# utiasASRL/mm_masking

Hardware: AMD Instinct MI355X
Metric: scan-pairs/s (mask-CNN + 10-iter dICP fwd+bwd) (higher is better)
Workload: dtype bf16; 1 GPU; BASELINE configs[2]: train_icp_weights step fwd+bwd, batch=32 per GPU, 10 dICP iters, point-to-plane Huber, dim=2; 400x3360 polar radar -> GO-CFAR + peaks + polar->Cartesian 640x640 -> U-Net (hand-written NHWC bf16 MFMA kernels, fp32 masters) -> dICP (fp32 points, fp64 normal equations) -> rot+trans+mask_pts loss -> Adam; batch_per_gpu=32, global_batch=32, scan_pts_pad=5120, map_pts=20000, map_pts_pad=20480, icp_iters=10, parallelism=dp1, scene_density=survey (SURVEY.md 8d: 3 500-5 000 valid scan points of 5 120)

## Files before the change

### include/mmk.h

```cpp
#ifndef MMK_H_
#define MMK_H_

#include <stddef.h>
#include <stdint.h>

#ifdef __cplusplus
extern "C" {
#endif

#define MMK_VERSION 502

#define MMK_OK 0
#define MMK_ERR_ARG (-1)
#define MMK_ERR_HIP (-2)
#define MMK_ERR_WORKSPACE (-3)

#define MMK_ICP_PT2PT 0
#define MMK_ICP_PT2PL 1

#define MMK_NN_BRUTE 0
#define MMK_NN_GRID 1

#define MMK_LOSS_NONE 0
#define MMK_LOSS_CAUCHY 1
// ... 175 lines not shown
int mmk_cfar_mask_p(const float *raw, int32_t B, int32_t A, int32_t R, int32_t w2, int32_t guard, int32_t mincol,
                    int32_t maxcol, const float *a_thresh, const float *b_thresh, int32_t per_scan, int32_t diff,
                    float steep_fact, float *mask, void *stream);

size_t mmk_cfar_mask_bwd_p_ws_bytes(int32_t B, int32_t A);
int mmk_cfar_mask_bwd_p(const float *raw, const float *grad_mask , int32_t B, int32_t A, int32_t R, int32_t w2,
                        int32_t guard, int32_t mincol, int32_t maxcol, const float *a_thresh, const float *b_thresh,
                        int32_t per_scan, float steep_fact, float *grad_raw , float *grad_a,
                        float *grad_b , void *workspace, size_t workspace_bytes, void *stream);

size_t mmk_extract_peaks_workspace_bytes(int32_t B, int32_t A, int32_t R, int32_t max_pts);
int mmk_extract_peaks(const float *mask, int32_t B, int32_t A, int32_t R, float res,
                      const float *azimuths , const float *times ,
                      const float *T_ab, int32_t diff, float steep_fact, int32_t max_pts,
                      float *out_pc, int32_t *out_count, void *workspace,
                      size_t workspace_bytes, void *stream);
size_t mmk_extract_peaks_bwd_workspace_bytes(int32_t B, int32_t A, int32_t R, int32_t max_pts);
int mmk_extract_peaks_bwd(const float *mask, int32_t B, int32_t A, int32_t R, float res, const float *azimuths ,
                          const float *T_ab, int32_t diff, float steep_fact, int32_t max_pts,
                          const float *grad_pc , float *grad_mask , void *workspace,
                          size_t workspace_bytes, void *stream);

int mmk_polar_to_cart(const float *polar, const float *azimuths ,
                      const float *range_grid, const float *angle_grid, int32_t B,
                      int32_t A, int32_t R, int32_t W, float radar_resolution,
                      int32_t interpolate_crossover, int32_t fix_wobble, float *cart,
                      void *stream);
int mmk_polar_to_cart_pair(const float *polar, const float *polar2, const float *azimuths,
                           const float *range_grid, const float *angle_grid, int32_t B, int32_t A,
                           int32_t R, int32_t W, float radar_resolution, int32_t interpolate_crossover,
                           int32_t fix_wobble, float *cart, float *cart2, void *stream);

int mmk_cart_to_polar(const double *cart, const double *sin_az, const double *cos_az, const double *range_coords,
                      int32_t B, int32_t A, int32_t R, int32_t H, int32_t W, double cart_resolution, double *polar,
                      void *stream);

size_t mmk_polar_to_cart_bwd_ws_bytes(int32_t B, int32_t A, int32_t R, int32_t W);
int mmk_polar_to_cart_bwd(const float *grad_cart , const float *azimuths , const float *range_grid,
                          const float *angle_grid, int32_t B, int32_t A, int32_t R, int32_t W, float radar_resolution,
                          int32_t interpolate_crossover, int32_t fix_wobble, float *grad_polar , void *ws,
                          size_t ws_bytes, void *stream);

size_t mmk_cart_to_polar_bwd_ws_bytes(int32_t B, int32_t A, int32_t R, int32_t H, int32_t W);
int mmk_cart_to_polar_bwd(const double *grad_polar , const double *sin_az, const double *cos_az,
                          const double *range_coords, int32_t B, int32_t A, int32_t R, int32_t H, int32_t W,
                          double radar_resolution, double cart_resolution, double *grad_cart , void *ws,
                          size_t ws_bytes, void *stream);

int mmk_mask_polar_scan(const float *scan , const float *mask_cart , const double *sin_az,
                        const double *cos_az, const double *range_coords, int32_t B, int32_t A, int32_t R, int32_t H,
                        int32_t W, double cart_resolution, float *out , void *stream);

size_t mmk_mask_polar_scan_bwd_ws_bytes(int32_t B, int32_t A, int32_t R, int32_t H, int32_t W);
int mmk_mask_polar_scan_bwd(const float *grad_out , const float *scan , const float *mask_cart ,
                            const double *sin_az, const double *cos_az, const double *range_coords, int32_t B, int32_t A,
                            int32_t R, int32_t H, int32_t W, double radar_resolution, double cart_resolution,
                            float *grad_scan , float *grad_mask , void *ws, size_t ws_bytes,
                            void *stream);

int mmk_sample_weights_fwd(const float *mask , const float *pc ,
                           int32_t B, int32_t N, int32_t pc_cols, int32_t H, int32_t W,
                           int32_t cart_pixel_width, float cart_resolution,
                           float *weights , void *stream);
size_t mmk_sample_weights_bwd_ws_bytes(int32_t B, int32_t N);
int mmk_sample_weights_bwd(const float *grad_weights , const float *pc, int32_t B,
                           int32_t N, int32_t pc_cols, int32_t H, int32_t W,
                           int32_t cart_pixel_width, float cart_resolution, float *grad_mask,
                           void *ws, size_t ws_bytes, void *stream);
int mmk_sample_weights_bwd_pc(const float *grad_weights , const float *mask , const float *pc,
                              int32_t B, int32_t N, int32_t pc_cols, int32_t H, int32_t W,
                              int32_t cart_pixel_width, float cart_resolution, float *grad_pc, void *stream);

int mmk_sample_weights_polar_fwd(const float *mask , const float *pc , const float *azimuths ,
                                 int32_t B, int32_t N, int32_t pc_cols, int32_t A, int32_t R, float radar_resolution,
                                 int32_t interpolate_crossover, int32_t fix_wobble, float *weights , void *stream);
size_t mmk_sample_weights_polar_bwd_ws_bytes(int32_t B, int32_t N);
int mmk_sample_weights_polar_bwd(const float *grad_weights , const float *pc, const float *azimuths, int32_t B, int32_t N,
                                 int32_t pc_cols, int32_t A, int32_t R, float radar_resolution, int32_t interpolate_crossover,
                                 int32_t fix_wobble, float *grad_mask , void *ws, size_t ws_bytes, void *stream);
int mmk_sample_weights_polar_bwd_pc(const float *grad_weights , const float *mask , const float *pc,
                                    const float *azimuths, int32_t B, int32_t N, int32_t pc_cols, int32_t A, int32_t R,
                                    float radar_resolution, int32_t interpolate_crossover, int32_t fix_wobble,
                                    float *grad_pc , void *stream);

int mmk_host_read_rows(const char *path, int64_t header_bytes, int32_t rows, int32_t row_bytes, int32_t col0,
                       int32_t ncols, int32_t roll, void *dst);
typedef struct mmk_read_job {
    const char *path;
    int64_t header_bytes;
    int32_t rows, row_bytes, col0, ncols, roll, reserved;
    void *dst;
} mmk_read_job;
int mmk_host_read_rows_batch(const mmk_read_job *jobs, int32_t n_jobs, int32_t threads);
int mmk_u8_to_float(const void *in , const float *lut256, int64_t n, float *out, void *stream);

int mmk_weight_stats(const float *weights , const float *pc , int32_t B, int32_t N,
                     int32_t pc_cols, float *partial, float *out, void *stream);

int mmk_bev_raster(const float *pc , int32_t B, int32_t M, int32_t pc_cols,
                   int32_t W, float cart_resolution, float *bev , void *stream);

typedef struct {
    const void *x1;
    const void *x2;
    int32_t C1, C2;
    const void *wpack;
    const float *bias;
    void *y1;
    const void *relu_src1;
    int32_t O1, accumulate1;
    float scale1;
    void *y2;
    const void *relu_src2;
    int32_t O2, accumulate2;
    float scale2;
    int32_t B, H, W;
    int32_t relu;
    float leaky_slope;
    float drop_p;
    uint32_t seed;
    void *pool_y;
    void *pool_arg;
    const void *x1_pool_arg;
    float x1_pool_scale;
} mmk_conv_desc;

size_t mmk_conv_desc_bytes(void);
int32_t mmk_conv3x3_pool_fusable(int32_t cin, int32_t cout, int32_t B, int32_t H, int32_t W);

size_t mmk_conv3x3_packed_elems(int32_t cout, int32_t cin, int32_t transposed);
int mmk_conv3x3_pack_weights(const float *W, int32_t cout, int32_t cin, int32_t transposed,
                             void *packed, void *stream);
int mmk_conv3x3_pack_weights_batch(int32_t n, const float *const *W, const int32_t *cout, const int32_t *cin,
                                   int32_t transposed, void *const *packed, void *stream);
int mmk_conv3x3(const mmk_conv_desc *d, void *stream);
int32_t mmk_conv3x3_wgrad_slices(int32_t cout, int32_t cin, int32_t c1, int32_t B, int32_t H, int32_t W);
int mmk_conv3x3_wgrad_partial(const void *x1, const void *x2, int32_t C1, int32_t C2, const void *g, int32_t cout,
                              int32_t B, int32_t H, int32_t W, float *partials, int32_t accumulate, void *stream);

int mmk_conv_bwd_fused(const void *x, const void *g, const void *wpack_t, float scale, int32_t B, int32_t H, int32_t W,
                       int32_t C, void *dx, float *partials, int32_t accumulate, void *stream);
int mmk_conv_bwd_fused_pooled(const void *x, const void *gy, const void *arg, float pool_scale, const void *wpack_t, float scale,
                              int32_t B, int32_t H, int32_t W, int32_t C, void *dx, float *partials, int32_t accumulate,
                              void *stream);
int mmk_conv3x3_wgrad_partial_pooled(const void *x1, const void *x2, int32_t C1, int32_t C2, const void *gy, const void *arg,
                                     float pool_scale, int32_t cout, int32_t B, int32_t H, int32_t W, float *partials,
                                     int32_t accumulate, void *stream);

int mmk_conv8x16_bwd_fused(const void *x, const void *g, const void *wpack_t, float scale, int32_t B, int32_t H, int32_t W,
                           void *dx, float *partials, int32_t accumulate, void *stream);

int mmk_conv16x8_bwd_fused(const void *x1, const void *x2, const void *g, const void *wpack_t, float scale, int32_t B, int32_t H,
                           int32_t W, void *dx1, void *dx2, float *partials, int32_t accumulate, void *stream);
int mmk_conv3x3_wgrad_unpack_batch(int32_t n, const float *const *src, const int32_t *slices, const int32_t *cout,
                                   const int32_t *cin, float *const *dW, float *const *db, void *stream);

int mmk_channel_minmax(const float *x , int32_t B, int32_t C, int64_t hw, float *part,
                       float *pre , float *minmax , void *stream);
int mmk_channel_meanstd(const float *x , int32_t B, int32_t C, int64_t hw, double *part,
                        float *pre , void *stream);
int mmk_conv_first(const float *x, int32_t cin, const float *W, const float *bias, const float *pre,
                   int32_t B, int32_t H, int32_t Wd, float leaky_slope, void *y, void *stream);
size_t mmk_conv_first_wgrad_ws_bytes(int32_t cin);
int mmk_conv_first_wgrad(const float *x, int32_t cin, const void *g, const float *pre, int32_t B,
                         int32_t H, int32_t Wd, float *dW, float *db, float *ws, size_t ws_bytes, void *stream);
#define MMK_NORM_NONE 0
#define MMK_NORM_MINMAX 1
#define MMK_NORM_STANDARDIZE 2
size_t mmk_conv_first_dgrad_ws_bytes(int32_t cin);
int mmk_conv_first_dgrad(const void *g, int32_t cin, const float *W, const float *x , const float *pre ,
                         const float *minmax , int32_t B, int32_t H, int32_t Wd, float *grad_x, void *ws ,
                         size_t ws_bytes, void *stream);
int mmk_input_norm_bwd(float *grad_x, const float *x, int32_t cin, const float *pre, const float *minmax ,
                       int32_t mode, int32_t B, int32_t H, int32_t Wd, const void *ws, size_t ws_bytes, void *stream);

int mmk_maxpool2_fwd(const void *x, int32_t B, int32_t H, int32_t W, int32_t C, void *y, void *stream);
int mmk_maxpool2_bwd(const void *d, const void *gy, int32_t B, int32_t H, int32_t W, int32_t C, float scale,
                     float leaky_slope, void *gz, void *stream);
int mmk_maxpool2_fwd_arg(const void *x, int32_t B, int32_t H, int32_t W, int32_t C, void *y, void *arg, void *stream);
int mmk_maxpool2_bwd_arg(const void *arg, const void *gy, int32_t B, int32_t H, int32_t W, int32_t C, float scale,
                         void *gz, void *stream);

int mmk_upsample_fwd(const void *x, int32_t B, int32_t Hs, int32_t Ws, int32_t C, int32_t Ho, int32_t Wo, void *y,
                     void *stream);
int mmk_upsample_bwd(const void *gy, int32_t B, int32_t Hs, int32_t Ws, int32_t C, int32_t Ho, int32_t Wo,
                     const void *relu_src, float scale, float leaky_slope, void *gx, void *stream);

#define MMK_FINAL_BWD_WS_FLOATS 16384
int mmk_final_fwd(const void *x, const float *w, const float *bias, int64_t npix, float *mask, void *stream);
int mmk_final_bwd(const void *x, const float *w, const float *mask, const float *gmask, int64_t npix, float scale,
                  float leaky_slope, void *gx, float *dW, float *db, float *ws, void *stream);
int mmk_mask_normalize(const float *mask , int32_t B, int64_t npix_per, float *part,
                       float *mask_n, float *amax, void *stream);
int mmk_final_bwd_normalized(const void *x, const float *w, const float *mask, const float *mask_n,
                             const float *amax, const float *gmask_n, int32_t B, int64_t npix_per,
                             float scale, float leaky_slope, float *part, float *coef, void *gx, float *dW,
                             float *db, float *ws, void *stream);

int mmk_bn_forward_stats(const void *a, int64_t npix, int32_t C, const float *gamma, const float *beta, float eps,
                         float momentum, float *running_mean, float *running_var, float *part, float *stat,
                         float *affine, void *stream);
int mmk_bn_apply(const void *a, int64_t npix, int32_t C, const float *affine, float drop_p, uint32_t seed, void *y,
                 void *stream);
int mmk_bn_backward(const void *gd, const void *d, float drop_scale, const void *a, int64_t npix, int32_t C,
                    const float *stat, const float *affine, const float *gamma, float leaky_slope, int32_t accumulate,
                    float *part, float *coef, float *dgamma, float *dbeta, void *gz, void *stream);

typedef struct {
    int32_t B, H, W, cin;
    const float *x;
    const float *pre;
    const float *const *params;
    float drop_p;
    uint32_t seed;
    float leaky_slope;
    int32_t norm;
    void *workspace;
    size_t workspace_bytes;
    float *mask;
    int32_t keep_full_res;
} mmk_unet_desc;

size_t mmk_unet_workspace_bytes(int32_t B, int32_t H, int32_t W, int32_t cin);
size_t mmk_unet_scratch_bytes(int32_t B, int32_t H, int32_t W, int32_t cin);
int mmk_unet_forward(const mmk_unet_desc *d, void *stream);
int mmk_unet_backward(const mmk_unet_desc *d, const float *gmask, float *const *grads, void *scratch,
                      size_t scratch_bytes, void *stream);
#define MMK_UNET_GRAD_BUCKETS 3
int32_t mmk_unet_grad_bucket(int32_t bucket, int32_t *first_param, int32_t *n_params);
int mmk_unet_backward_buckets(const mmk_unet_desc *d, const float *gmask, float *const *grads, void *scratch,
                              size_t scratch_bytes, void *const *bucket_events, void *stream);
int mmk_unet_backward_input(const mmk_unet_desc *d, const float *gmask, float *const *grads, float *grad_x, int32_t norm_mode,
                            const float *minmax, void *scratch, size_t scratch_bytes, void *const *bucket_events, void *stream);
int mmk_unet_tensor(int32_t B, int32_t H, int32_t W, int32_t cin, int32_t id, size_t *offset, int32_t *h,
                    int32_t *w, int32_t *c);

#ifdef __cplusplus
}
#endif
#endif
```

### mm_masking_amd/_lib.py

```python
import ctypes
import os
import sys
import subprocess

import torch

_HERE = os.path.dirname(os.path.abspath(__file__))
_ROOT = os.path.dirname(_HERE)
SO_PATH = os.environ.get("MMK_LIB", os.path.join(_HERE, "libmmk_hip.so"))
SOURCES = ["mmk_api.hip", "mmk_icp.hip", "mmk_radar.hip", "mmk_unet.hip", "mmk_unet_driver.hip", "mmk_loader.hip", "mmk_loss.hip"]

_lib = None

c_f32p = ctypes.c_void_p
c_vp = ctypes.c_void_p


class MmkError(RuntimeError):
    pass


class ReadJob(ctypes.Structure):
    _fields_ = [("path", ctypes.c_char_p), ("header_bytes", ctypes.c_int64), ("rows", ctypes.c_int32),
                ("row_bytes", ctypes.c_int32), ("col0", ctypes.c_int32), ("ncols", ctypes.c_int32), ("roll", ctypes.c_int32),
                ("reserved", ctypes.c_int32), ("dst", ctypes.c_void_p)]


class IcpParams(ctypes.Structure):
    _fields_ = [("B", ctypes.c_int32), ("N", ctypes.c_int32), ("M", ctypes.c_int32),
                ("tgt_cols", ctypes.c_int32), ("dim", ctypes.c_int32), ("icp_type", ctypes.c_int32),
                ("loss", ctypes.c_int32), ("loss_k", ctypes.c_float), ("trim_dist", ctypes.c_float),
                ("tolerance", ctypes.c_float), ("max_iter", ctypes.c_int32), ("save_state", ctypes.c_int32),
                ("check_every", ctypes.c_int32), ("nn_method", ctypes.c_int32),
                ("trim_steep", ctypes.c_float)]


class IcpSoft(ctypes.Structure):
    _fields_ = [("k", ctypes.c_int32), ("temp", ctypes.c_float)]


class ConvDesc(ctypes.Structure):
    _fields_ = [("x1", ctypes.c_void_p), ("x2", ctypes.c_void_p), ("C1", ctypes.c_int32), ("C2", ctypes.c_int32),
                ("wpack", ctypes.c_void_p), ("bias", ctypes.c_void_p),
                ("y1", ctypes.c_void_p), ("relu_src1", ctypes.c_void_p), ("O1", ctypes.c_int32),
                ("accumulate1", ctypes.c_int32), ("scale1", ctypes.c_float),
                ("y2", ctypes.c_void_p), ("relu_src2", ctypes.c_void_p), ("O2", ctypes.c_int32),
                ("accumulate2", ctypes.c_int32), ("scale2", ctypes.c_float),
                ("B", ctypes.c_int32), ("H", ctypes.c_int32), ("W", ctypes.c_int32), ("relu", ctypes.c_int32),
                ("leaky_slope", ctypes.c_float), ("drop_p", ctypes.c_float), ("seed", ctypes.c_uint32), ("pool_y", ctypes.c_void_p),
                ("pool_arg", ctypes.c_void_p), ("x1_pool_arg", ctypes.c_void_p), ("x1_pool_scale", ctypes.c_float)]


class UNetDesc(ctypes.Structure):
    _fields_ = [("B", ctypes.c_int32), ("H", ctypes.c_int32), ("W", ctypes.c_int32), ("cin", ctypes.c_int32),
                ("x", ctypes.c_void_p), ("pre", ctypes.c_void_p), ("params", ctypes.POINTER(ctypes.c_void_p)),
                ("drop_p", ctypes.c_float), ("seed", ctypes.c_uint32), ("leaky_slope", ctypes.c_float), ("norm", ctypes.c_int32),
                ("workspace", ctypes.c_void_p), ("workspace_bytes", ctypes.c_size_t), ("mask", ctypes.c_void_p),
                ("keep_full_res", ctypes.c_int32)]


FINAL_BWD_WS_FLOATS = 16384
NORM_MODES = {None: 0, "none": 0, "minmax": 1, "standardize": 2}
ICP_TYPES = {"pt2pt": 0, "pt2pl": 1}
LOSSES = {None: 0, "none": 0, "l2": 0, "cauchy": 1, "huber": 2, "geman_mcclure": 3, "welsch": 4}
NN_METHODS = {"brute": 0, "grid": 1}


def build(verbose=False):
    from concurrent.futures import ThreadPoolExecutor
    csrc = os.path.join(_HERE, "csrc")
    srcs = [os.path.join(csrc, s) for s in SOURCES]
    common = [os.path.join(csrc, "mmk_common.h"), os.path.join(csrc, "mmk_unet_shared.h"), os.path.join(_ROOT, "include", "mmk.h")]
    incs = [os.path.join(csrc, f) for f in sorted(os.listdir(csrc)) if f.endswith(".inc")]
    extra = {"mmk_unet.hip": incs, "mmk_loader.hip": incs}
    objdir = os.path.join(csrc, "_obj")
    os.makedirs(objdir, exist_ok=True)
    hipcc = os.environ.get("HIPCC", "/opt/rocm/bin/hipcc")
    flags = ["--offload-arch=gfx950", "-O3", "-std=c++17", "-fPIC", "-ffp-contract=off", "-I", os.path.join(_ROOT, "include")]
    per_file = {"mmk_unet.hip": ["-mllvm", "-amdgpu-mfma-vgpr-form"]}
    jobs, objs = [], []
    for src in srcs:
        obj = os.path.join(objdir, os.path.basename(src)[:-4] + ".o")
        objs.append(obj)
        deps = [src] + common + extra.get(os.path.basename(src), []) + [os.path.abspath(__file__)]
        if not (os.path.exists(obj) and all(os.path.getmtime(obj) >= os.path.getmtime(d) for d in deps)):
            jobs.append([hipcc] + flags + per_file.get(os.path.basename(src), []) + ["-c", src, "-o", obj])
    if not jobs and os.path.exists(SO_PATH) and all(os.path.getmtime(SO_PATH) >= os.path.getmtime(o) for o in objs):
        return SO_PATH

    def run(cmd):
        if verbose:
            print(" ".join(cmd), flush=True)
        try:
            subprocess.check_call(cmd)
        except subprocess.CalledProcessError:
            plain = [c for c in cmd if c not in sum(per_file.values(), [])]
            if len(plain) == len(cmd):
                raise
            print("libmmk_hip: retrying without %s" % " ".join(sorted(set(cmd) - set(plain))), file=sys.stderr, flush=True)
            subprocess.check_call(plain)
    with ThreadPoolExecutor(max_workers=max(1, min(len(jobs), os.cpu_count() or 1))) as ex:
        list(ex.map(run, jobs))
    run([hipcc, "--offload-arch=gfx950", "-shared", "-fPIC", "-o", SO_PATH] + objs)
    return SO_PATH


def _declare(lib):
    i32, f32, sz = ctypes.c_int32, ctypes.c_float, ctypes.c_size_t
    P = ctypes.POINTER(IcpParams)
    S = ctypes.POINTER(IcpSoft)
    sig = {
        "mmk_version": (ctypes.c_int, []),
        "mmk_last_error": (ctypes.c_char_p, []),
        "mmk_icp_params_bytes": (sz, []),
        "mmk_icp_workspace_bytes": (sz, [P]),
        "mmk_icp_forward": (ctypes.c_int, [P] + [c_vp] * 10 + [c_vp, sz, ctypes.POINTER(ctypes.c_int), c_vp]),
        "mmk_icp_backward": (ctypes.c_int, [P] + [c_vp] * 11 + [c_vp, sz, c_vp]),
        "mmk_icp_backward_points_workspace_bytes": (sz, [P, i32]),
        "mmk_icp_backward_points": (ctypes.c_int, [P] + [c_vp] * 13 + [c_vp, sz, c_vp]),
        "mmk_icp_status": (ctypes.c_int, [P, c_vp, sz, c_vp, c_vp]),
        "mmk_icp_forward_hp": (ctypes.c_int, [P] + [c_vp] * 10 + [c_vp, i32, c_vp, sz, ctypes.POINTER(ctypes.c_int), c_vp]),
        "mmk_icp_backward_hp_workspace_bytes": (sz, [P, i32, i32]),
        "mmk_icp_backward_hp": (ctypes.c_int, [P] + [c_vp] * 13 + [c_vp, i32, c_vp, c_vp, sz, c_vp]),
        "mmk_icp_soft_workspace_bytes": (sz, [P, S]),
        "mmk_icp_forward_soft": (ctypes.c_int, [P] + [c_vp] * 10 + [S, c_vp, sz, ctypes.POINTER(ctypes.c_int), c_vp]),
        "mmk_icp_backward_soft_workspace_bytes": (sz, [P, S, i32]),
        "mmk_icp_backward_soft": (ctypes.c_int, [P] + [c_vp] * 13 + [S, c_vp, sz, c_vp]),
        "mmk_icp_forward_soft_t": (ctypes.c_int, [P] + [c_vp] * 10 + [S, c_vp, i32, c_vp, sz, ctypes.POINTER(ctypes.c_int), c_vp]),
        "mmk_icp_backward_soft_t_workspace_bytes": (sz, [P, S, i32, i32]),
        "mmk_icp_backward_soft_t": (ctypes.c_int, [P] + [c_vp] * 13 + [S, c_vp, i32, c_vp, c_vp, sz, c_vp]),
        "mmk_knn_search_workspace_bytes": (sz, [i32, i32, i32, i32]),
        "mmk_knn_search": (ctypes.c_int, [c_vp, c_vp, c_vp, i32, i32, i32, i32, i32, i32, c_vp, c_vp, c_vp, sz, c_vp]),
        "mmk_pose_loss_fwd": (ctypes.c_int, [c_vp, i32, c_vp, c_vp]),
        "mmk_pose_loss_bwd": (ctypes.c_int, [c_vp, i32, c_vp, c_vp, c_vp, c_vp]),
        "mmk_bce_ws_bytes": (sz, []),
        "mmk_bce_mean_fwd": (ctypes.c_int, [c_vp, c_vp, ctypes.c_int64, c_vp, sz, c_vp, c_vp]),
        "mmk_bce_mean_bwd": (ctypes.c_int, [c_vp, c_vp, ctypes.c_int64, c_vp, c_vp, c_vp]),
        "mmk_pose_loss_gt_fwd": (ctypes.c_int, [c_vp, c_vp, i32, c_vp, c_vp]),
        "mmk_pose_loss_gt_bwd": (ctypes.c_int, [c_vp, c_vp, i32, c_vp, c_vp, c_vp, c_vp]),
        "mmk_val_metric": (ctypes.c_int, [c_vp, c_vp, i32, c_vp, c_vp]),
        "mmk_fft_threshold_ws_bytes": (sz, [i32]),
        "mmk_fft_threshold_mask": (ctypes.c_int, [c_vp, i32, ctypes.c_int64, c_vp, sz, c_vp, c_vp]),
        "mmk_bce_fft_threshold_fwd": (ctypes.c_int, [c_vp, c_vp, i32, ctypes.c_int64, c_vp, sz, c_vp, c_vp, c_vp]),
        "mmk_bce_fft_threshold_bwd": (ctypes.c_int, [c_vp, c_vp, i32, ctypes.c_int64, c_vp, c_vp, c_vp, c_vp]),
        "mmk_icp_partials_count": (sz, [P]),
        "mmk_icp_accumulate": (ctypes.c_int, [P] + [c_vp] * 8 + [c_vp]),
        "mmk_icp_solve_update": (ctypes.c_int, [P] + [c_vp] * 7 + [c_vp]),
        "mmk_nn_padded_m": (i32, [i32]),
        "mmk_pack_target": (ctypes.c_int, [c_vp, i32, i32, i32, i32, c_vp, c_vp]),
        "mmk_nn_workspace_bytes": (sz, [i32, i32, i32, i32]),
        "mmk_nn_search": (ctypes.c_int, [c_vp, c_vp, c_vp, i32, i32, i32, i32, c_vp, c_vp, c_vp, sz, c_vp]),
        "mmk_knn_normals_workspace_bytes": (sz, [i32, i32]),
        "mmk_knn_normals": (ctypes.c_int, [c_vp, i32, i32, i32, i32, i32, f32, f32, c_vp, c_vp, c_vp, c_vp, c_vp, c_vp, sz, c_vp]),
        "mmk_nn_profile_begin": (ctypes.c_int, [i32]),
        "mmk_nn_profile_end": (ctypes.c_int, [ctypes.POINTER(ctypes.c_float), i32, ctypes.POINTER(ctypes.c_int32)]),
        "mmk_conv3x3_packed_elems": (sz, [i32, i32, i32]),
        "mmk_conv3x3_pack_weights": (ctypes.c_int, [c_vp, i32, i32, i32, c_vp, c_vp]),
        "mmk_conv3x3_pack_weights_batch": (ctypes.c_int, [i32, c_vp, c_vp, c_vp, i32, c_vp, c_vp]),
        "mmk_conv3x3": (ctypes.c_int, [ctypes.POINTER(ConvDesc), c_vp]),
        "mmk_conv3x3_wgrad_unpack_batch": (ctypes.c_int, [i32, c_vp, c_vp, c_vp, c_vp, c_vp, c_vp, c_vp]),
        "mmk_conv3x3_wgrad_slices": (i32, [i32, i32, i32, i32, i32, i32]),
        "mmk_conv3x3_wgrad_partial": (ctypes.c_int, [c_vp, c_vp, i32, i32, c_vp, i32, i32, i32, i32, c_vp, i32, c_vp]),
        "mmk_conv_bwd_fused": (ctypes.c_int, [c_vp, c_vp, c_vp, ctypes.c_float, i32, i32, i32, i32, c_vp, c_vp, i32, c_vp]),
        "mmk_conv_bwd_fused_pooled": (ctypes.c_int, [c_vp, c_vp, c_vp, f32, c_vp, f32, i32, i32, i32, i32, c_vp, c_vp, i32, c_vp]),
        "mmk_conv3x3_wgrad_partial_pooled": (ctypes.c_int, [c_vp, c_vp, i32, i32, c_vp, c_vp, f32, i32, i32, i32, i32, c_vp, i32, c_vp]),
        "mmk_conv8x16_bwd_fused": (ctypes.c_int, [c_vp, c_vp, c_vp, ctypes.c_float, i32, i32, i32, c_vp, c_vp, i32, c_vp]),
        "mmk_conv16x8_bwd_fused": (ctypes.c_int, [c_vp, c_vp, c_vp, c_vp, ctypes.c_float, i32, i32, i32, c_vp, c_vp, c_vp, i32, c_vp]),
        "mmk_conv_desc_bytes": (sz, []),
        "mmk_conv3x3_pool_fusable": (ctypes.c_int32, [i32, i32, i32, i32, i32]),
        "mmk_channel_minmax": (ctypes.c_int, [c_vp, i32, i32, ctypes.c_int64, c_vp, c_vp, c_vp, c_vp]),
        "mmk_channel_meanstd": (ctypes.c_int, [c_vp, i32, i32, ctypes.c_int64, c_vp, c_vp, c_vp]),
        "mmk_conv_first": (ctypes.c_int, [c_vp, i32, c_vp, c_vp, c_vp, i32, i32, i32, f32, c_vp, c_vp]),
        "mmk_conv_first_wgrad_ws_bytes": (sz, [i32]),
        "mmk_conv_first_wgrad": (ctypes.c_int, [c_vp, i32, c_vp, c_vp, i32, i32, i32, c_vp, c_vp, c_vp, sz, c_vp]),
        "mmk_conv_first_dgrad_ws_bytes": (sz, [i32]),
        "mmk_conv_first_dgrad": (ctypes.c_int, [c_vp, i32, c_vp, c_vp, c_vp, c_vp, i32, i32, i32, c_vp, c_vp, sz, c_vp]),
        "mmk_input_norm_bwd": (ctypes.c_int, [c_vp, c_vp, i32, c_vp, c_vp, i32, i32, i32, i32, c_vp, sz, c_vp]),
        "mmk_maxpool2_fwd": (ctypes.c_int, [c_vp, i32, i32, i32, i32, c_vp, c_vp]),
        "mmk_maxpool2_bwd": (ctypes.c_int, [c_vp, c_vp, i32, i32, i32, i32, f32, f32, c_vp, c_vp]),
        "mmk_maxpool2_fwd_arg": (ctypes.c_int, [c_vp, i32, i32, i32, i32, c_vp, c_vp, c_vp]),
        "mmk_maxpool2_bwd_arg": (ctypes.c_int, [c_vp, c_vp, i32, i32, i32, i32, f32, c_vp, c_vp]),
        "mmk_upsample_fwd": (ctypes.c_int, [c_vp, i32, i32, i32, i32, i32, i32, c_vp, c_vp]),
        "mmk_upsample_bwd": (ctypes.c_int, [c_vp, i32, i32, i32, i32, i32, i32, c_vp, f32, f32, c_vp, c_vp]),
        "mmk_final_fwd": (ctypes.c_int, [c_vp, c_vp, c_vp, ctypes.c_int64, c_vp, c_vp]),
        "mmk_final_bwd": (ctypes.c_int, [c_vp, c_vp, c_vp, c_vp, ctypes.c_int64, f32, f32, c_vp, c_vp, c_vp, c_vp, c_vp]),
        "mmk_mask_normalize": (ctypes.c_int, [c_vp, i32, ctypes.c_int64, c_vp, c_vp, c_vp, c_vp]),
        "mmk_final_bwd_normalized": (ctypes.c_int, [c_vp, c_vp, c_vp, c_vp, c_vp, c_vp, i32, ctypes.c_int64, f32, f32, c_vp, c_vp,
                                                    c_vp, c_vp, c_vp, c_vp, c_vp]),
        "mmk_bn_forward_stats": (ctypes.c_int, [c_vp, ctypes.c_int64, i32, c_vp, c_vp, f32, f32, c_vp, c_vp, c_vp, c_vp, c_vp, c_vp]),
        "mmk_bn_apply": (ctypes.c_int, [c_vp, ctypes.c_int64, i32, c_vp, f32, ctypes.c_uint32, c_vp, c_vp]),
        "mmk_bn_backward": (ctypes.c_int, [c_vp, c_vp, f32, c_vp, ctypes.c_int64, i32, c_vp, c_vp, c_vp, f32, i32, c_vp, c_vp, c_vp,
                                           c_vp, c_vp, c_vp]),
        "mmk_unet_workspace_bytes": (sz, [i32, i32, i32, i32]),
        "mmk_unet_scratch_bytes": (sz, [i32, i32, i32, i32]),
        "mmk_unet_forward": (ctypes.c_int, [ctypes.POINTER(UNetDesc), c_vp]),
        "mmk_unet_backward": (ctypes.c_int, [ctypes.POINTER(UNetDesc), c_vp, ctypes.POINTER(ctypes.c_void_p), c_vp, sz, c_vp]),
        "mmk_unet_backward_buckets": (ctypes.c_int, [ctypes.POINTER(UNetDesc), c_vp, ctypes.POINTER(ctypes.c_void_p), c_vp, sz,
                                                     ctypes.POINTER(ctypes.c_void_p), c_vp]),
        "mmk_unet_backward_input": (ctypes.c_int, [ctypes.POINTER(UNetDesc), c_vp, ctypes.POINTER(ctypes.c_void_p), c_vp, i32, c_vp,
                                                   c_vp, sz, ctypes.POINTER(ctypes.c_void_p), c_vp]),
        "mmk_unet_grad_bucket": (i32, [i32, ctypes.POINTER(i32), ctypes.POINTER(i32)]),
        "mmk_unet_tensor": (ctypes.c_int, [i32, i32, i32, i32, i32, ctypes.POINTER(sz), ctypes.POINTER(i32), ctypes.POINTER(i32),
                                           ctypes.POINTER(i32)]),
        "mmk_cfar_mask": (ctypes.c_int, [c_vp, i32, i32, i32, i32, i32, i32, i32, f32, f32, i32, f32, c_vp, c_vp]),
        "mmk_cfar_mask_bwd": (ctypes.c_int, [c_vp, c_vp, i32, i32, i32, i32, i32, i32, i32, f32, f32, f32, c_vp, c_vp]),
        "mmk_cfar_mask_p": (ctypes.c_int, [c_vp, i32, i32, i32, i32, i32, i32, i32, c_vp, c_vp, i32, i32, f32, c_vp, c_vp]),
        "mmk_cfar_mask_bwd_p_ws_bytes": (sz, [i32, i32]),
        "mmk_cfar_mask_bwd_p": (ctypes.c_int, [c_vp, c_vp, i32, i32, i32, i32, i32, i32, i32, c_vp, c_vp, i32, f32, c_vp, c_vp, c_vp,
                                               c_vp, sz, c_vp]),
        "mmk_extract_peaks_workspace_bytes": (sz, [i32, i32, i32, i32]),
        "mmk_extract_peaks_bwd_workspace_bytes": (sz, [i32, i32, i32, i32]),
        "mmk_extract_peaks_bwd": (ctypes.c_int, [c_vp, i32, i32, i32, f32, c_vp, c_vp, i32, f32, i32, c_vp, c_vp, c_vp, sz, c_vp]),
        "mmk_extract_peaks": (ctypes.c_int, [c_vp, i32, i32, i32, f32, c_vp, c_vp, c_vp, i32, f32, i32, c_vp, c_vp,
                                             c_vp, sz, c_vp]),
        "mmk_polar_to_cart": (ctypes.c_int, [c_vp, c_vp, c_vp, c_vp, i32, i32, i32, i32, f32, i32, i32, c_vp, c_vp]),
        "mmk_polar_to_cart_pair": (ctypes.c_int, [c_vp, c_vp, c_vp, c_vp, c_vp, i32, i32, i32, i32, f32, i32, i32, c_vp, c_vp,
                                                  c_vp]),
        "mmk_cart_to_polar": (ctypes.c_int, [c_vp, c_vp, c_vp, c_vp, i32, i32, i32, i32, i32, ctypes.c_double, c_vp, c_vp]),
        "mmk_polar_to_cart_bwd_ws_bytes": (sz, [i32, i32, i32, i32]),
        "mmk_polar_to_cart_bwd": (ctypes.c_int, [c_vp, c_vp, c_vp, c_vp, i32, i32, i32, i32, f32, i32, i32, c_vp, c_vp, sz, c_vp]),
        "mmk_cart_to_polar_bwd_ws_bytes": (sz, [i32, i32, i32, i32, i32]),
        "mmk_cart_to_polar_bwd": (ctypes.c_int, [c_vp, c_vp, c_vp, c_vp, i32, i32, i32, i32, i32, ctypes.c_double, ctypes.c_double,
                                                 c_vp, c_vp, sz, c_vp]),
        "mmk_mask_polar_scan": (ctypes.c_int, [c_vp, c_vp, c_vp, c_vp, c_vp, i32, i32, i32, i32, i32, ctypes.c_double, c_vp, c_vp]),
        "mmk_mask_polar_scan_bwd_ws_bytes": (sz, [i32, i32, i32, i32, i32]),
        "mmk_mask_polar_scan_bwd": (ctypes.c_int, [c_vp, c_vp, c_vp, c_vp, c_vp, c_vp, i32, i32, i32, i32, i32, ctypes.c_double,
                                                   ctypes.c_double, c_vp, c_vp, c_vp, sz, c_vp]),
        "mmk_sample_weights_fwd": (ctypes.c_int, [c_vp, c_vp, i32, i32, i32, i32, i32, i32, f32, c_vp, c_vp]),
        "mmk_host_read_rows": (ctypes.c_int, [ctypes.c_char_p, ctypes.c_int64, i32, i32, i32, i32, i32, c_vp]),
        "mmk_host_read_rows_batch": (ctypes.c_int, [ctypes.POINTER(ReadJob), i32, i32]),
        "mmk_u8_to_float": (ctypes.c_int, [c_vp, c_vp, ctypes.c_int64, c_vp, c_vp]),
        "mmk_sample_weights_bwd_ws_bytes": (sz, [i32, i32]),
        "mmk_sample_weights_bwd": (ctypes.c_int, [c_vp, c_vp, i32, i32, i32, i32, i32, i32, f32, c_vp, c_vp, sz, c_vp]),
        "mmk_sample_weights_bwd_pc": (ctypes.c_int, [c_vp, c_vp, c_vp, i32, i32, i32, i32, i32, i32, f32, c_vp, c_vp]),
        "mmk_sample_weights_polar_fwd": (ctypes.c_int, [c_vp, c_vp, c_vp, i32, i32, i32, i32, i32, f32, i32, i32, c_vp, c_vp]),
        "mmk_sample_weights_polar_bwd_ws_bytes": (sz, [i32, i32]),
        "mmk_sample_weights_polar_bwd": (ctypes.c_int, [c_vp, c_vp, c_vp, i32, i32, i32, i32, i32, f32, i32, i32, c_vp, c_vp, sz,
                                                        c_vp]),
        "mmk_sample_weights_polar_bwd_pc": (ctypes.c_int, [c_vp, c_vp, c_vp, c_vp, i32, i32, i32, i32, i32, f32, i32, i32, c_vp,
                                                           c_vp]),
        "mmk_weight_stats": (ctypes.c_int, [c_vp, c_vp, i32, i32, i32, c_vp, c_vp, c_vp]),
        "mmk_bev_raster": (ctypes.c_int, [c_vp, i32, i32, i32, i32, f32, c_vp, c_vp]),
    }
    for name, (res, args) in sig.items():
        fn = getattr(lib, name)
        fn.restype = res
        fn.argtypes = args
    return sig


EXPORTED = None


def lib():
    global _lib, EXPORTED
    if _lib is None:
        if not os.path.exists(SO_PATH):
            raise MmkError("libmmk_hip.so is not built: run `python -c 'import __graft_entry__ as g; g.build()'` "
                           "(hipcc --offload-arch=gfx950).  The HIP path has no CPU fallback.")
        try:
            loaded = ctypes.CDLL(SO_PATH)
        except OSError as e:
            raise MmkError("cannot load %s: %s" % (SO_PATH, e)) from e
        EXPORTED = _declare(loaded)
        if loaded.mmk_conv_desc_bytes() != ctypes.sizeof(ConvDesc):
            raise MmkError("%s: mmk_conv_desc is %d bytes, the ctypes mirror %d" % (SO_PATH, loaded.mmk_conv_desc_bytes(), ctypes.sizeof(ConvDesc)))
        if loaded.mmk_icp_params_bytes() != ctypes.sizeof(IcpParams):
            raise MmkError("%s: mmk_icp_params is %d bytes, the ctypes mirror %d" % (SO_PATH, loaded.mmk_icp_params_bytes(), ctypes.sizeof(IcpParams)))
        _lib = loaded
    return _lib


def check(rc):
    if rc != 0:
        raise MmkError("libmmk_hip: %s (code %d)" % (lib().mmk_last_error().decode(errors="replace"), rc))


def stream_ptr(device=None):
    if device is not None:
        idx = device.index if isinstance(device, torch.device) else int(device)
        if idx is not None and idx != torch.cuda.current_device():
            raise MmkError("tensors live on cuda:%d but the current HIP device is cuda:%d: call torch.cuda.set_device() "
                           "(one process per GPU) or wrap the call in `with torch.cuda.device(...)`"
                           % (idx, torch.cuda.current_device()))
    return ctypes.c_void_p(torch.cuda.current_stream(device).cuda_stream)


def ptr(t, dtype=None, name="tensor"):
    if t is None:
        return ctypes.c_void_p(0)
    if not t.is_cuda:
        raise MmkError("%s must live on a HIP device (got %s); the kernels have no CPU path" % (name, t.device))
    if dtype is not None and t.dtype != dtype:
        raise MmkError("%s must be %s (got %s)" % (name, dtype, t.dtype))
    if not t.is_contiguous():
        raise MmkError("%s must be contiguous" % name)
    return ctypes.c_void_p(t.data_ptr())


_ws_cache = {}


def workspace(nbytes, device, tag):
    key = (device.index, torch.cuda.current_stream(device).cuda_stream, tag)
    buf = _ws_cache.get(key)
    if buf is None or buf.numel() < nbytes:
        buf = torch.empty(max(int(nbytes), 1), dtype=torch.uint8, device=device)
        _ws_cache[key] = buf
    return buf


def dev_f32(t, device):
    return t.detach().to(device=device, dtype=torch.float32).contiguous()
```

### mm_masking_amd/csrc/mmk_unet.hip

```cpp
#include <math.h>
#include <stdlib.h>

#include <algorithm>
#include <type_traits>

#include "mmk_common.h"
#include "mmk_unet_shared.h"

namespace {

using namespace mmku;

__device__ __forceinline__ unsigned cvt_pk_bf16(float lo, float hi)
{
    unsigned r;
    asm("v_cvt_pk_bf16_f32 %0, %1, %2" : "=v"(r) : "v"(lo), "v"(hi));
    return r;
}
__device__ __forceinline__ unsigned pk_relu_bf16(unsigned x)
{
    unsigned r;
    asm("v_pk_max_i16 %0, %1, 0" : "=v"(r) : "v"(x));
    return r;
}
// ... 1634 lines not shown
        {
            if (t + t_step < t_end) {
                ld_tx += adv_tx;
                const int cx = ld_tx >= tiles_x ? 1 : 0;
                ld_tx -= cx ? tiles_x : 0;
                ld_ty += adv_ty + cx;
                const int cy = ld_ty >= tiles_y ? 1 : 0;
                ld_ty -= cy ? tiles_y : 0;
                ld_b += adv_b + cy;
            }
            load_tile(ld_b, ld_ty, ld_tx);
        }
        i32x2 fa[2][2 * MT], fb[2][2 * NTW];
#define WG_ISSUE(R, BUF)                                                                                 \
    {                                                                                                    \
        _Pragma("unroll") for (int m = 0; m < MT; ++m) {                                                 \
            fa[BUF][2 * m] = (m == 0) ? tr_read_o<((R) * TW * PG) * 2>(g_ad)                             \
                           : (m == 1) ? tr_read_o<((R) * TW * PG + 16) * 2>(g_ad)                        \
                           : (m == 2) ? tr_read_o<((R) * TW * PG + 32) * 2>(g_ad)                        \
                                      : tr_read_o<((R) * TW * PG + 48) * 2>(g_ad);                       \
            fa[BUF][2 * m + 1] = (m == 0) ? tr_read_o<((R) * TW * PG + 16 * PG) * 2>(g_ad)                \
                               : (m == 1) ? tr_read_o<((R) * TW * PG + 16 + 16 * PG) * 2>(g_ad)           \
                               : (m == 2) ? tr_read_o<((R) * TW * PG + 32 + 16 * PG) * 2>(g_ad)           \
                                          : tr_read_o<((R) * TW * PG + 48 + 16 * PG) * 2>(g_ad);          \
        }                                                                                                \
        _Pragma("unroll") for (int n = 0; n < NTW; ++n) {                                                \
            fb[BUF][2 * n] = tr_read_o<((R) * WT * PK) * 2>(b_ad[n]);                                    \
            fb[BUF][2 * n + 1] = tr_read_o<((R) * WT * PK + 16 * PK) * 2>(b_ad[n]);                       \
        }                                                                                                \
    }
#define WG_CONSUME(BUF)                                                                                  \
    {                                                                                                    \
        _Pragma("unroll") for (int m = 0; m < MT; ++m) {                                                 \
            const bf16x8 af = frag_from(fa[BUF][2 * m], fa[BUF][2 * m + 1]);                             \
             \
             \
            _Pragma("unroll") for (int n = 0; n < NTW; ++n)                                              \
                acc[m][n] = __builtin_amdgcn_mfma_f32_16x16x32_bf16(af, frag_from(fb[BUF][2 * n], fb[BUF][2 * n + 1]), acc[m][n], 0, 0, 0); \
            accb[m] = __builtin_amdgcn_mfma_f32_16x16x32_bf16(af, ones, accb[m], 0, 0, 0);               \
        }                                                                                                \
    }
#define WG_STEP(R)                                                                                       \
    {                                                                                                    \
        asm volatile("s_waitcnt lgkmcnt(0)" ::: "memory");                                               \
        __builtin_amdgcn_sched_barrier(0);                                                               \
        if ((R) + 1 < TH) WG_ISSUE(((R) + 1 < TH ? (R) + 1 : 0), ((R) + 1) & 1);                         \
        __builtin_amdgcn_sched_barrier(0);                                                               \
        WG_CONSUME((R) & 1);                                                                             \
    }
        WG_ISSUE(0, 0);
        WG_STEP(0) WG_STEP(1) WG_STEP(2) WG_STEP(3) WG_STEP(4) WG_STEP(5) WG_STEP(6) WG_STEP(7)
        static_assert(TH == 8, "WG_STEP expansion above covers 8 tile rows");
#undef WG_STEP
#undef WG_CONSUME
#undef WG_ISSUE
    }

    const size_t pstride = (size_t)9 * a.COUT * a.CIN + a.COUT;
#pragma unroll
    for (int m = 0; m < MT; ++m) {
#pragma unroll
        for (int rr = 0; rr < 4; ++rr) {
            const int co = group * CM + m * 16 + g4 * 4 + rr;
            if (co >= a.COUT) continue;
#pragma unroll
            for (int n = 0; n < NTW; ++n) {
                const int nt = wv + 4 * n;
                if (nt >= NTT) continue;
                int tap, ci;
                if (CK >= 16) {
                    tap = nt / (CK / 16);
                    ci = chunk * CK + (nt % (CK / 16)) * 16 + i16;
                } else {
                    tap = 2 * nt + (i16 >> 3);
                    ci = i16 & 7;
                }
                if (tap < 9) {
                    float *d = a.partials + (size_t)blockIdx.x * pstride + ((size_t)tap * a.COUT + co) * a.CIN + ci;
                    *d = a.acc_partials ? *d + acc[m][n][rr] : acc[m][n][rr];
                }
            }
            if (wv == 0 && chunk == 0 && i16 == 0) {
                float *d = a.partials + (size_t)blockIdx.x * pstride + (size_t)9 * a.COUT * a.CIN + co;
                *d = a.acc_partials ? *d + accb[m][rr] : accb[m][rr];
            }
        }
    }
}

constexpr size_t wgrad_smem(int CX, int CG)
{
    return ((size_t)(HT * WT + 8) * wg_pitch(CX) + (size_t)(TH * TW + 8) * wg_pitch(CG)) * sizeof(bf16);
}

template <int CK, int CM, bool G8>
int wgrad_spatial(int cout, int cin, int B, int H, int W)
{
    constexpr int cap = (CK <= 16 && CM == 16) ? 4 : 8;
    int per_cu = 0;
    if (blocks_per_cu<conv3x3_wgrad_kernel<CK, CM, G8>>(CONV_THREADS, wgrad_smem(CK, G8 ? 8 : CM), cap, &per_cu) != hipSuccess) return -1;
    const int tiles = ((W + TW - 1) / TW) * ((H + TH - 1) / TH) * B;
    const int chunks = cin / CK, groups = (cout + CM - 1) / CM;
    int spatial = (256 * per_cu) / (chunks * groups);
    spatial = spatial < 1 ? 1 : (spatial > tiles ? tiles : spatial);
    return spatial >= 8 ? (spatial & ~7) : spatial;
}

template <int CK, int CM, bool G8, bool POOLG = false>
int launch_wgrad(const WgradArgs &a, hipStream_t st)
{
    constexpr size_t smem = wgrad_smem(CK, G8 ? 8 : CM);
    const int spatial = wgrad_spatial<CK, CM, G8>(a.COUT, a.CIN, a.B, a.H, a.W);
    if (spatial < 1) {
        mmk::set_error("mmk_conv3x3_wgrad: occupancy query failed");
        return MMK_ERR_HIP;
    }
    const int chunks = a.CIN / CK, groups = (a.COUT + CM - 1) / CM;
    if constexpr (POOLG)
        MMK_CHECK_HIP((raise_lds_limit<conv3x3_wgrad_kernel<CK, CM, G8, true>>(smem > 64 * 1024, smem)));
    hipLaunchKernelGGL((conv3x3_wgrad_kernel<CK, CM, G8, POOLG>), dim3(spatial, chunks, groups), dim3(CONV_THREADS), smem, st, a);
    MMK_LAUNCH_CHECK();
    return MMK_OK;
}


struct BwdFusedArgs {
    const bf16 *x, *x2;
    const bf16 *g;
    const bf16 *wpack_t;
    bf16 *dx, *dx2;
    float scale;
    int masked;
    int accumulate_dx;
    int B, H, W;
    float *partials;
    int acc_partials;
    const unsigned *g_arg = nullptr;
    float g_scale = 1.f;
};

BwdFusedArgs bwd_fused_args(const void *x, const void *x2, const void *g, const void *wpack_t, void *dx, void *dx2, float scale,
                            int masked, int B, int H, int W, float *partials, int accumulate)
{
    BwdFusedArgs a = {};
    a.x = (const bf16 *)x; a.x2 = (const bf16 *)x2; a.g = (const bf16 *)g; a.wpack_t = (const bf16 *)wpack_t;
    a.dx = (bf16 *)dx; a.dx2 = (bf16 *)dx2; a.scale = scale; a.masked = masked;
    a.B = B; a.H = H; a.W = W; a.partials = partials; a.acc_partials = accumulate;
    return a;
}

template <int CX, int CG, bool POOLG = false>
__global__ __launch_bounds__(CONV_THREADS) void conv_bwd_fused_kernel(const BwdFusedArgs a)
{
    static_assert((CX == 8 || CX == 16) && (CG == 8 || CG == 16), "thin layers");
    constexpr int NTT = CX == 8 ? 5 : 9;
    constexpr int NTW = (NTT + 3) / 4;
    constexpr int NS = CG == 8 ? 3 : 5;
    constexpr int NT = 4;
    constexpr int GX = CX / 8, GG = CG / 8;
    __shared__ __attribute__((aligned(16))) bf16 x_tile[(HT * WT + 8) * CX];
    __shared__ __attribute__((aligned(16))) bf16 g_tile[(HT * WT + 8) * CG];
    __shared__ __attribute__((aligned(16))) bf16 w_lds[NS * 64 * 8];

    const int tid = threadIdx.x, lane = tid & 63;
    const int wv = __builtin_amdgcn_readfirstlane(tid >> 6);
    const int tiles_x = (a.W + TW - 1) / TW, tiles_y = (a.H + TH - 1) / TH;
    const int tpi = tiles_x * tiles_y;
    const int total_tiles = tpi * a.B;
    const int i16 = lane & 15, g4 = lane >> 4, q = i16 >> 2, pp = i16 & 3;
    const bool split = a.x2 != nullptr;

    f32x4 acc[NTW], accb = {0.f, 0.f, 0.f, 0.f};
#pragma unroll
    for (int n = 0; n < NTW; ++n) acc[n] = (f32x4){0.f, 0.f, 0.f, 0.f};
    bf16x8 ones;
#pragma unroll
    for (int j = 0; j < 8; ++j) ones[j] = (bf16)1.0f;
    unsigned b_ad[NTW];
#pragma unroll
    for (int n = 0; n < NTW; ++n) {
        const int nt = wv + 4 * n;
        int tap = CX == 8 ? 2 * nt + (pp >> 1) : nt;
        const int col = CX == 8 ? 4 * (pp & 1) : 4 * pp;
        tap = tap > 8 ? 8 : tap;
        const int ty = tap / 3, tx = tap % 3;
        b_ad[n] = lds_addr(x_tile) + (unsigned)((((ty * WT) + 4 * g4 + q + tx) * CX + col) * 2);
    }
    const unsigned g_ad = lds_addr(g_tile) + (unsigned)(((WT + 1 + 4 * g4 + q) * CG + 4 * pp) * 2);

    int d_lane[NS];
#pragma unroll
    for (int ks = 0; ks < NS; ++ks) {
        int tap = CG == 8 ? 4 * ks + (lane >> 4) : 2 * ks + (lane >> 5);
        const int ch = CG == 8 ? 0 : 8 * ((lane >> 4) & 1);
        tap = tap > 8 ? 8 : tap;
        d_lane[ks] = ((2 * wv + tap / 3) * WT + (lane & 15) + tap % 3) * CG + ch;
    }
    const int n8 = lane >> 4;
    const int lrow8 = 2 * wv + (n8 >> 1), lcol8 = (n8 & 1) * 16 + (lane & 15);
    const int lpix8 = lrow8 * a.W + lcol8;
    const int s_off8 = ((lrow8 + 1) * WT + lcol8 + 1) * CX;
    int o_pix[NT], s_off[NT];
#pragma unroll
    for (int n = 0; n < NT; ++n) {
        const int r = 2 * wv + (n >> 1), c = (n & 1) * 16 + (lane & 15);
        o_pix[n] = r * a.W + c;
        s_off[n] = ((r + 1) * WT + c + 1) * CX + (lane >> 4) * 4;
    }
    bf16 *const o_base = (a.dx2 != nullptr) ? ((lane >> 5) ? a.dx2 : a.dx) + ((lane >> 4) & 1) * 4 : a.dx + (lane >> 4) * 4;
    const int o_stride = (a.dx2 != nullptr) ? 8 : 16;
    for (int i = tid; i < NS * 64; i += CONV_THREADS) reinterpret_cast<u32x4 *>(w_lds)[i] = reinterpret_cast<const u32x4 *>(a.wpack_t)[i];

    constexpr int NX = HT * WT * GX, NG = HT * WT * GG;
    constexpr int RX = (NX + CONV_THREADS - 1) / CONV_THREADS, RG = (NG + CONV_THREADS - 1) / CONV_THREADS;
    constexpr int PH = TH / 2 + 2, PW = TW / 2 + 2, NPG = PH * PW * GG;
    constexpr int NRG = POOLG ? (NPG + CONV_THREADS - 1) / CONV_THREADS : RG;
    u32x4 rx[RX], rg[NRG];
    unsigned rc[POOLG ? NRG : 1];
    const int Hp = a.H >> 1, Wp = a.W >> 1;
    auto load_tile = [&](int b, int tyi, int txi) {
        int tv = tid;
        asm volatile("" : "+v"(tv));
        const int tx0 = txi * TW, ty0 = tyi * TH;
        const int pix0 = (b * a.H + ty0) * a.W + tx0;
#pragma unroll
        for (int i = 0; i < RX; ++i) {
            int gi = tv + i * CONV_THREADS;
            gi = gi < NX ? gi : NX - 1;
            const int pix = gi / GX, half = gi % GX;
            const int dy = pix / WT - 1, dx = pix % WT - 1;
            const bool ok = (unsigned)(ty0 + dy) < (unsigned)a.H && (unsigned)(tx0 + dx) < (unsigned)a.W;
            const long po = pix0 + dy * a.W + dx;
            const bf16 *src = split ? (half ? a.x2 : a.x) + po * 8 : a.x + po * CX + half * 8;
            rx[i] = *(ok ? reinterpret_cast<const u32x4 *>(src) : &g_zero16);
        }
        if constexpr (POOLG) {
#pragma unroll
            for (int i = 0; i < NRG; ++i) {
                int gi = tv + i * CONV_THREADS;
                gi = gi < NPG ? gi : NPG - 1;
                const int pp = gi / GG, gc = gi % GG;
                const int py = (ty0 >> 1) + pp / PW - 1, px = (tx0 >> 1) + pp % PW - 1;
                const bool ok = (unsigned)py < (unsigned)Hp && (unsigned)px < (unsigned)Wp;
                const long e = (long)((b * Hp + py) * Wp + px) * GG + gc;
                rg[i] = *(ok ? reinterpret_cast<const u32x4 *>(a.g + e * 8) : &g_zero16);
                rc[i] = *(ok ? a.g_arg + e : reinterpret_cast<const unsigned *>(&g_zero16));
            }
        } else {
#pragma unroll
            for (int i = 0; i < RG; ++i) {
                int gi = tv + i * CONV_THREADS;
                gi = gi < NG ? gi : NG - 1;
                const int pix = gi / GG, gc = gi % GG;
                const int dy = pix / WT - 1, dx = pix % WT - 1;
                const bool ok = (unsigned)(ty0 + dy) < (unsigned)a.H && (unsigned)(tx0 + dx) < (unsigned)a.W;
                rg[i] = *(ok ? reinterpret_cast<const u32x4 *>(a.g + (long)(pix0 + dy * a.W + dx) * CG + gc * 8) : &g_zero16);
            }
        }
    };
    auto store_tile = [&]() {
        int tv = tid;
        asm volatile("" : "+v"(tv));
#pragma unroll
        for (int i = 0; i < RX; ++i) {
            const int gi = tv + i * CONV_THREADS;
            if (gi < NX) *reinterpret_cast<u32x4 *>(x_tile + (size_t)gi * 8) = rx[i];
        }
        if constexpr (POOLG) {
#pragma unroll
            for (int i = 0; i < NRG; ++i) {
                const int gi = tv + i * CONV_THREADS;
                const int pp = gi / GG, gc = gi % GG;
                const int r0 = 2 * (pp / PW) - 1, c0 = 2 * (pp % PW) - 1;
                poolg_write(g_tile + (r0 * WT + c0) * CG + gc * 8, CG, WT * CG, r0, c0, HT, WT, gi < NPG, rg[i], rc[i], a.g_scale);
            }
        } else {
#pragma unroll
            for (int i = 0; i < RG; ++i) {
                const int gi = tv + i * CONV_THREADS;
                if (gi < NG) *reinterpret_cast<u32x4 *>(g_tile + (size_t)gi * 8) = rg[i];
            }
        }
    };

    int t_first, t_step, t_end;
    if ((gridDim.x & 7) == 0) {
        const int per_xcd = (total_tiles + 7) / 8;
        const int xcd = blockIdx.x & 7;
        t_first = xcd * per_xcd + ((int)blockIdx.x >> 3);
        t_step = (int)gridDim.x >> 3;
        t_end = min(total_tiles, (xcd + 1) * per_xcd);
    } else {
        t_first = blockIdx.x; t_step = gridDim.x; t_end = total_tiles;
    }
    const int adv_tx = t_step % tiles_x, adv_ty = (t_step / tiles_x) % tiles_y, adv_b = t_step / tpi;
    int ld_b = t_first / tpi, ld_ty = (t_first % tpi) / tiles_x, ld_tx = t_first % tiles_x;
    int cb = ld_b, cty = ld_ty, ctx = ld_tx;
    if (t_first < t_end) {
        load_tile(ld_b, ld_ty, ld_tx);
        store_tile();
    }
    __syncthreads();
    for (int t = t_first; t < t_end; t += t_step) {
        const int b = cb;
        const int tx0 = ctx * TW, ty0 = cty * TH;
        const int pix0 = (b * a.H + ty0) * a.W + tx0;
        const bool ok8 = (ty0 + lrow8) < a.H && (tx0 + lcol8) < a.W;
        u32x4 e8_acc = {0u, 0u, 0u, 0u};
        if constexpr (CX == 8) e8_acc = *((ok8 && a.accumulate_dx) ? reinterpret_cast<const u32x4 *>(a.dx + (long)(pix0 + lpix8) * 8) : &g_zero16);
        {
            if (t + t_step < t_end) {
                ld_tx += adv_tx;
                const int cx = ld_tx >= tiles_x ? 1 : 0;
                ld_tx -= cx ? tiles_x : 0;
                ld_ty += adv_ty + cx;
                const int cy = ld_ty >= tiles_y ? 1 : 0;
                ld_ty -= cy ? tiles_y : 0;
                ld_b += adv_b + cy;
            }
            load_tile(ld_b, ld_ty, ld_tx);
            cb = ld_b; cty = ld_ty; ctx = ld_tx;
        }
        i32x2 fa[2][2], fb[2][2 * NTW];
#define BF_ISSUE(R, BUF)                                                                     \
    {                                                                                        \
        fa[BUF][0] = tr_read_o<((R) * WT * CG) * 2>(g_ad);                                   \
        fa[BUF][1] = tr_read_o<((R) * WT * CG + 16 * CG) * 2>(g_ad);                         \
        _Pragma("unroll") for (int n = 0; n < NTW; ++n) {                                    \
            fb[BUF][2 * n] = tr_read_o<((R) * WT * CX) * 2>(b_ad[n]);                        \
            fb[BUF][2 * n + 1] = tr_read_o<((R) * WT * CX + 16 * CX) * 2>(b_ad[n]);          \
        }                                                                                    \
    }
#define BF_CONSUME(BUF)                                                                      \
    {                                                                                        \
        const bf16x8 af = frag_from(fa[BUF][0], fa[BUF][1]);                                 \
        _Pragma("unroll") for (int n = 0; n < NTW; ++n)                                      \
            acc[n] = __builtin_amdgcn_mfma_f32_16x16x32_bf16(af, frag_from(fb[BUF][2 * n], fb[BUF][2 * n + 1]), acc[n], 0, 0, 0); \
        accb = __builtin_amdgcn_mfma_f32_16x16x32_bf16(af, ones, accb, 0, 0, 0);             \
    }
#define BF_STEP(R)                                                                           \
    {                                                                                        \
        asm volatile("s_waitcnt lgkmcnt(0)" ::: "memory");                                   \
        __builtin_amdgcn_sched_barrier(0);                                                   \
        if ((R) + 1 < TH) BF_ISSUE(((R) + 1 < TH ? (R) + 1 : 0), ((R) + 1) & 1);             \
        __builtin_amdgcn_sched_barrier(0);                                                   \
        BF_CONSUME((R) & 1);                                                                 \
    }
        BF_ISSUE(0, 0);
        BF_STEP(0) BF_STEP(1) BF_STEP(2) BF_STEP(3) BF_STEP(4) BF_STEP(5) BF_STEP(6) BF_STEP(7)
        static_assert(TH == 8, "BF_STEP expansion above covers 8 tile rows");
#undef BF_STEP
#undef BF_CONSUME
#undef BF_ISSUE
        f32x4 dacc[NT];
#pragma unroll
        for (int n = 0; n < NT; ++n) dacc[n] = (f32x4){0.f, 0.f, 0.f, 0.f};
#pragma unroll
        for (int ks = 0; ks < NS; ++ks) {
            const bf16 *bl = g_tile + d_lane[ks];
            bf16x8 bf[NT];
#pragma unroll
            for (int n = 0; n < NT; ++n) bf[n] = *reinterpret_cast<const bf16x8 *>(bl + ((n >> 1) * WT + (n & 1) * 16) * CG);
            const bf16x8 af = *reinterpret_cast<const bf16x8 *>(w_lds + ((size_t)(ks * 64 + lane)) * 8);
#pragma unroll
            for (int n = 0; n < NT; ++n) dacc[n] = __builtin_amdgcn_mfma_f32_16x16x32_bf16(af, bf[n], dacc[n], 0, 0, 0);
        }
        u32x4 e8_src = {0u, 0u, 0u, 0u};
        bf16x4 e_src[NT];
        if constexpr (CX == 8) {
            e8_src = *reinterpret_cast<const u32x4 *>(x_tile + s_off8);
        } else {
#pragma unroll
            for (int n = 0; n < NT; ++n) e_src[n] = *reinterpret_cast<const bf16x4 *>(x_tile + s_off[n]);
        }
#pragma unroll
        for (int i = 0; i < RX; ++i) asm volatile("" : "+v"(rx[i]));
#pragma unroll
        for (int i = 0; i < NRG; ++i) asm volatile("" : "+v"(rg[i]));
        if constexpr (POOLG) {
#pragma unroll
            for (int i = 0; i < NRG; ++i) asm volatile("" : "+v"(rc[i]));
        }
        if constexpr (CX == 8) {
            float v8[8];
#pragma unroll
            for (int r = 0; r < 4; ++r) {
                const auto s01 = __builtin_amdgcn_permlane16_swap(__float_as_uint(dacc[0][r]), __float_as_uint(dacc[1][r]), false, false);
                const auto s23 = __builtin_amdgcn_permlane16_swap(__float_as_uint(dacc[2][r]), __float_as_uint(dacc[3][r]), false, false);
                const auto lo = __builtin_amdgcn_permlane32_swap(s01[0], s23[0], false, false);
                const auto hi = __builtin_amdgcn_permlane32_swap(s01[1], s23[1], false, false);
                v8[r] = __uint_as_float(lo[0]);
                v8[4 + r] = __uint_as_float(hi[0]);
            }
            float sv[8], av[8];
            unpack8(e8_src, sv);
            unpack8(e8_acc, av);
#pragma unroll
            for (int r = 0; r < 8; ++r) {
                const float v = fmaxf(v8[r] + 0.f, -INFINITY);
                const float masked = (sv[r] > 0.f) ? v * a.scale : 0.f;
                v8[r] = masked + av[r];
            }
            u32x4 *dst8 = ok8 ? reinterpret_cast<u32x4 *>(a.dx + (long)(pix0 + lpix8) * 8) : reinterpret_cast<u32x4 *>(g_sink16);
            *dst8 = pack8(v8);
        } else {
#pragma unroll
            for (int n = 0; n < NT; ++n) {
                const bool okp = (ty0 + 2 * wv + (n >> 1)) < a.H && (tx0 + (n & 1) * 16 + (lane & 15)) < a.W;
                bf16x4 outv;
#pragma unroll
                for (int r = 0; r < 4; ++r) {
                    const float v = fmaxf(dacc[n][r] + 0.f, -INFINITY);
                    const float masked = ((float)e_src[n][r] > 0.f) ? v * a.scale : 0.f;
                    outv[r] = (bf16)(a.masked ? masked + 0.f : v);
                }
                bf16x4 *dst = okp ? reinterpret_cast<bf16x4 *>(o_base + (long)(pix0 + o_pix[n]) * o_stride) : reinterpret_cast<bf16x4 *>(g_sink16);
                *dst = outv;
            }
        }
        if (t + t_step >= t_end) break;
        __syncthreads();
        store_tile();
        __syncthreads();
    }

    constexpr size_t pstride = (size_t)9 * CG * CX + CG;
#pragma unroll
    for (int rr = 0; rr < 4; ++rr) {
        const int co = g4 * 4 + rr;
        if (co >= CG) continue;
#pragma unroll
        for (int n = 0; n < NTW; ++n) {
            const int nt = wv + 4 * n;
            if (nt >= NTT) continue;
            const int tap = CX == 8 ? 2 * nt + (i16 >> 3) : nt;
            const int ci = CX == 8 ? (i16 & 7) : i16;
            if (tap < 9) {
                float *d = a.partials + (size_t)blockIdx.x * pstride + ((size_t)tap * CG + co) * CX + ci;
                *d = a.acc_partials ? *d + acc[n][rr] : acc[n][rr];
            }
        }
        if (wv == 0 && i16 == 0) {
            float *d = a.partials + (size_t)blockIdx.x * pstride + (size_t)9 * CG * CX + co;
            *d = a.acc_partials ? *d + accb[rr] : accb[rr];
        }
    }
}

constexpr int WGD_THREADS = 512;

template <bool POOLG = false>
__global__ __launch_bounds__(WGD_THREADS) void conv3x3_wgrad_deep_kernel(const WgradArgs a)
{
    constexpr int CK = 64, CM = 64, PK = wg_pitch(64), PG = wg_pitch(64);
    extern __shared__ __attribute__((aligned(16))) unsigned char smem[];
    bf16 *x_tile = reinterpret_cast<bf16 *>(smem);
    bf16 *g_tile = x_tile + (HT * WT + 8) * PK;

    const int tid = threadIdx.x, lane = tid & 63;
    const int wv = __builtin_amdgcn_readfirstlane(tid >> 6);
    const int wm = wv >> 2, wc = wv & 3;
    const int chunk = blockIdx.y, group = blockIdx.z;
    const int tiles_x = (a.W + TW - 1) / TW, tiles_y = (a.H + TH - 1) / TH;
    const int tpi = tiles_x * tiles_y;
    const int total_tiles = tpi * a.B;
    const int i16 = lane & 15, g4 = lane >> 4, q = i16 >> 2, pp = i16 & 3;

    f32x4 acc[3][3][2];
    f32x4 accb[2];
#pragma unroll
    for (int m = 0; m < 2; ++m) {
        accb[m] = (f32x4){0.f, 0.f, 0.f, 0.f};
#pragma unroll
        for (int ty = 0; ty < 3; ++ty)
#pragma unroll
            for (int tx = 0; tx < 3; ++tx) acc[ty][tx][m] = (f32x4){0.f, 0.f, 0.f, 0.f};
    }
    bf16x8 ones;
#pragma unroll
    for (int j = 0; j < 8; ++j) ones[j] = (bf16)1.0f;

    const unsigned xb0 = lds_addr(x_tile) + (unsigned)(((4 * g4 + q) * PK + wc * 16 + 4 * pp) * 2);
    const unsigned gb0 = lds_addr(g_tile) + (unsigned)(((4 * g4 + q) * PG + wm * 32 + 4 * pp) * 2);

    constexpr int GPP = CK / 8;
    constexpr int NIN = HT * WT * GPP;
    constexpr int RIN = (NIN + WGD_THREADS - 1) / WGD_THREADS;
    constexpr int GPG = CM / 8;
    constexpr int NG = TH * TW * GPG;
    constexpr int RG = (NG + WGD_THREADS - 1) / WGD_THREADS;
    constexpr int PWG = TW / 2, NPG = (TH / 2) * PWG * GPG;
    constexpr int NRG = POOLG ? (NPG + WGD_THREADS - 1) / WGD_THREADS : RG;
    u32x4 rin[RIN], rg[NRG];
    unsigned rc[POOLG ? NRG : 1];
    const int Hp = a.H >> 1, Wp = a.W >> 1;
    auto load_tile = [&](int b, int tyi, int txi) {
        int tv = tid;
        asm volatile("" : "+v"(tv));
        const int tx0 = txi * TW, ty0 = tyi * TH;
        const int c0 = chunk * CK;
        const bool in1 = c0 < a.C1;
        const bf16 *xb = in1 ? a.x1 : a.x2;
        const int xc = in1 ? a.C1 : a.C2, cb = in1 ? c0 : c0 - a.C1;
#pragma unroll
        for (int i = 0; i < RIN; ++i) {
            int gi = tv + i * WGD_THREADS;
            gi = gi < NIN ? gi : NIN - 1;
            const int pix = gi / GPP, gc = gi % GPP;
            const int yy = ty0 + pix / WT - 1, xx = tx0 + pix % WT - 1;
            const bool ok = yy >= 0 && yy < a.H && xx >= 0 && xx < a.W;
            const size_t p = ((size_t)b * a.H + yy) * a.W + xx;
            const u32x4 *sp = ok ? reinterpret_cast<const u32x4 *>(xb + p * xc + cb + gc * 8) : &g_zero16;
            rin[i] = *sp;
        }
        if constexpr (POOLG) {
#pragma unroll
            for (int i = 0; i < NRG; ++i) {
                int gi = tv + i * WGD_THREADS;
                gi = gi < NPG ? gi : NPG - 1;
                const int pp = gi / GPG, gc = gi % GPG;
                const int py = (ty0 >> 1) + pp / PWG, px = (tx0 >> 1) + pp % PWG;
                const bool ok = py < Hp && px < Wp;
                const size_t e = (((size_t)b * Hp + py) * Wp + px) * (a.COUT >> 3) + ((group * CM) >> 3) + gc;
                rg[i] = *(ok ? reinterpret_cast<const u32x4 *>(a.g + e * 8) : &g_zero16);
                rc[i] = *(ok ? a.g_arg + e : reinterpret_cast<const unsigned *>(&g_zero16));
            }
        } else {
#pragma unroll
        for (int i = 0; i < RG; ++i) {
            int gi = tv + i * WGD_THREADS;
            gi = gi < NG ? gi : NG - 1;
            const int pix = gi / GPG, gc = gi % GPG;
            const int yy = ty0 + pix / TW, xx = tx0 + pix % TW;
            const bool ok = yy < a.H && xx < a.W;
            const size_t p = ((size_t)b * a.H + yy) * a.W + xx;
            const u32x4 *sp = ok ? reinterpret_cast<const u32x4 *>(a.g + p * a.COUT + group * CM + gc * 8) : &g_zero16;
            rg[i] = *sp;
        }
        }
    };
    auto store_tile = [&]() {
        int tv = tid;
        asm volatile("" : "+v"(tv));
#pragma unroll
        for (int i = 0; i < RIN; ++i) {
            const int gi = tv + i * WGD_THREADS;
            if (gi < NIN) *reinterpret_cast<u32x4 *>(x_tile + (size_t)(gi / GPP) * PK + (gi % GPP) * 8) = rin[i];
        }
        if constexpr (POOLG) {
#pragma unroll
            for (int i = 0; i < NRG; ++i) {
                const int gi = tv + i * WGD_THREADS;
                const int pp = gi / GPG, gc = gi % GPG;
                const int r0 = 2 * (pp / PWG), c0 = 2 * (pp % PWG);
                poolg_write(g_tile + (r0 * TW + c0) * PG + gc * 8, PG, TW * PG, r0, c0, TH, TW, gi < NPG, rg[i], rc[i], a.g_scale);
            }
        } else {
#pragma unroll
        for (int i = 0; i < RG; ++i) {
            const int gi = tv + i * WGD_THREADS;
            if (gi < NG) *reinterpret_cast<u32x4 *>(g_tile + (size_t)(gi / GPG) * PG + (gi % GPG) * 8) = rg[i];
        }
        }
    };

    int t_first, t_step, t_end;
    if ((gridDim.x & 7) == 0) {
        const int per_xcd = (total_tiles + 7) / 8;
        const int xcd = blockIdx.x & 7;
        t_first = xcd * per_xcd + ((int)blockIdx.x >> 3);
        t_step = (int)gridDim.x >> 3;
        t_end = min(total_tiles, (xcd + 1) * per_xcd);
    } else {
        t_first = blockIdx.x; t_step = gridDim.x; t_end = total_tiles;
    }
    const int adv_tx = t_step % tiles_x, adv_ty = (t_step / tiles_x) % tiles_y, adv_b = t_step / tpi;
    int ld_b = t_first / tpi, ld_ty = (t_first % tpi) / tiles_x, ld_tx = t_first % tiles_x;
    if (t_first < t_end) load_tile(ld_b, ld_ty, ld_tx);
    for (int t = t_first; t < t_end; t += t_step) {
        __syncthreads();
        store_tile();
        __syncthreads();
        {
            if (t + t_step < t_end) {
                ld_tx += adv_tx;
                const int cx = ld_tx >= tiles_x ? 1 : 0;
                ld_tx -= cx ? tiles_x : 0;
                ld_ty += adv_ty + cx;
                const int cy = ld_ty >= tiles_y ? 1 : 0;
                ld_ty -= cy ? tiles_y : 0;
                ld_b += adv_b + cy;
            }
            load_tile(ld_b, ld_ty, ld_tx);
        }
        i32x2 fb[2][3][2], fa[4][2][2];
#define WGD_ISSUE(RHO)                                                                                   \
    {                                                                                                    \
// ... 1531 lines not shown

bool chan_ok(int c) { return c == 8 || c == 16 || c == 32 || (c >= 64 && c % 64 == 0); }

}

#ifdef MMK_DEEP_STAMPS
extern "C" int mmk_debug_deep_stamps(unsigned long long *buf)
{
    MMK_CHECK_HIP(hipMemcpyToSymbol(HIP_SYMBOL(g_deep_stamp_buf), &buf, sizeof(buf)));
    return MMK_OK;
}
#endif

extern "C" size_t mmk_conv3x3_packed_elems(int32_t cout, int32_t cin, int32_t transposed)
{
    const int co_n = transposed ? cin : cout, ci_n = transposed ? cout : cin;
    if (!chan_ok(co_n) || !chan_ok(ci_n)) return 0;
    const int CK = conv_ck(ci_n), CM = conv_cm(ci_n, co_n);
    const int groups = (co_n + CM - 1) / CM, chunks = ci_n / CK;
    return (size_t)groups * chunks * ksteps(CK) * (CM / 16) * 512;
}

extern "C" int mmk_conv3x3_pack_weights(const float *W, int32_t cout, int32_t cin, int32_t transposed, void *packed,
                                        void *stream)
{
    MMK_REQUIRE(W && packed, "mmk_conv3x3_pack_weights: NULL pointer");
    const size_t total = mmk_conv3x3_packed_elems(cout, cin, transposed);
    MMK_REQUIRE(total > 0, "mmk_conv3x3_pack_weights: unsupported channel counts %d -> %d", cin, cout);
    hipLaunchKernelGGL(pack_conv_weights_kernel, dim3((unsigned)((total + 255) / 256)), dim3(256), 0, (hipStream_t)stream, W,
                       cout, cin, transposed, (bf16 *)packed, (int)total);
    MMK_LAUNCH_CHECK();
    return MMK_OK;
}

extern "C" int mmk_conv3x3_pack_weights_batch(int32_t n, const float *const *W, const int32_t *cout, const int32_t *cin,
                                              int32_t transposed, void *const *packed, void *stream)
{
    MMK_REQUIRE(n >= 1 && W && cout && cin && packed, "mmk_conv3x3_pack_weights_batch: bad argument");
    for (int base = 0; base < n; base += PACK_BATCH_MAX) {
        PackBatch pb;
        const int m = std::min(PACK_BATCH_MAX, n - base);
        size_t most = 0;
        for (int i = 0; i < PACK_BATCH_MAX; ++i) {
            const int k = base + (i < m ? i : 0);
            MMK_REQUIRE(W[k] && packed[k], "mmk_conv3x3_pack_weights_batch: NULL pointer (layer %d)", k);
            const size_t total = mmk_conv3x3_packed_elems(cout[k], cin[k], transposed);
            MMK_REQUIRE(total > 0 && total < ((size_t)1 << 31), "mmk_conv3x3_pack_weights_batch: unsupported channel counts %d -> %d",
                        cin[k], cout[k]);
            pb.W[i] = W[k]; pb.out[i] = (bf16 *)packed[k]; pb.cout[i] = cout[k]; pb.cin[i] = cin[k];
            pb.total[i] = (int)total;
            most = std::max(most, total);
        }
        pb.transposed = transposed;
        const unsigned bx = (unsigned)std::min<size_t>((most + 255) / 256, 256);
        hipLaunchKernelGGL(pack_conv_weights_batch_kernel, dim3(bx, m), dim3(256), 0, (hipStream_t)stream, pb);
        MMK_LAUNCH_CHECK();
    }
    return MMK_OK;
}

extern "C" int mmk_conv3x3(const mmk_conv_desc *d, void *stream)
{
    MMK_REQUIRE(d != nullptr, "mmk_conv3x3: NULL descriptor");
    MMK_REQUIRE(d->x1 && d->wpack && (d->y1 || (d->pool_y && d->pool_arg)), "mmk_conv3x3: NULL pointer");
    MMK_REQUIRE(d->pool_arg == nullptr || d->pool_y != nullptr, "mmk_conv3x3: pool_arg needs pool_y");
    MMK_REQUIRE(d->B >= 1 && d->H >= 1 && d->W >= 1, "mmk_conv3x3: bad shape");
    const int cin = d->C1 + d->C2, cout = d->O1 + d->O2;
    MMK_REQUIRE(d->C1 % 8 == 0 && d->C2 % 8 == 0 && (d->C2 == 0 || d->x2), "mmk_conv3x3: bad input split %d+%d", d->C1, d->C2);
    MMK_REQUIRE(d->O1 % 8 == 0 && d->O2 % 8 == 0 && (d->O2 == 0 || d->y2), "mmk_conv3x3: bad output split %d+%d", d->O1, d->O2);
    MMK_REQUIRE(chan_ok(cin) && chan_ok(cout), "mmk_conv3x3: unsupported channel counts %d -> %d", cin, cout);
    MMK_REQUIRE(dropout_prob_ok(d->drop_p), "mmk_conv3x3: dropout probability %g out of range (it is quantised to thr / 65536, thr <= 65535)", (double)d->drop_p);
    ConvArgs a;
    a.x1 = (const bf16 *)d->x1; a.x2 = (const bf16 *)d->x2; a.C1 = d->C1; a.C2 = d->C2;
    a.wpack = (const bf16 *)d->wpack; a.bias = d->bias;
    a.o1 = {(bf16 *)d->y1, (const bf16 *)d->relu_src1, d->O1, d->accumulate1, d->scale1};
    a.o2 = {(bf16 *)d->y2, (const bf16 *)d->relu_src2, d->O2, d->accumulate2, d->scale2};
    a.B = d->B; a.H = d->H; a.W = d->W; a.CIN = cin; a.COUT = cout;
    MMK_REQUIRE(d->leaky_slope >= 0.f && d->leaky_slope <= 1.f, "mmk_conv3x3: leaky_slope must be in [0, 1]");
    a.relu = d->relu; a.slope = d->leaky_slope; a.drop_p = d->drop_p; a.seed = d->seed;
    a.pool_y = (bf16 *)d->pool_y;
    a.pool_arg = (unsigned char *)d->pool_arg;
    a.x1_pool_arg = (const unsigned *)d->x1_pool_arg;
    a.x1_pool_scale = d->x1_pool_scale;
    return dispatch_conv(a, (hipStream_t)stream);
}

extern "C" size_t mmk_conv_desc_bytes(void) { return sizeof(mmk_conv_desc); }

extern "C" int32_t mmk_conv3x3_pool_fusable(int32_t cin, int32_t cout, int32_t B, int32_t H, int32_t W)
{
    return pool_fusable(cin, cout, B, H, W) ? 1 : 0;
}

extern "C" int mmk_conv3x3_wgrad_unpack_batch(int32_t n, const float *const *src, const int32_t *slices, const int32_t *cout,
                                              const int32_t *cin, float *const *dW, float *const *db, void *stream)
{
    MMK_REQUIRE(n >= 1 && src && cout && cin && dW, "mmk_conv3x3_wgrad_unpack_batch: bad argument");
    for (int base = 0; base < n; base += PACK_BATCH_MAX) {
        UnpackBatch ub;
        const int m = std::min(PACK_BATCH_MAX, n - base);
        int most = 0;
        for (int i = 0; i < PACK_BATCH_MAX; ++i) {
            const int k = base + (i < m ? i : 0);
            MMK_REQUIRE(src[k] && dW[k] && cout[k] >= 1 && cin[k] >= 1, "mmk_conv3x3_wgrad_unpack_batch: bad layer %d", k);
            ub.src[i] = src[k]; ub.dW[i] = dW[k]; ub.cout[i] = cout[k]; ub.cin[i] = cin[k];
            ub.slices[i] = slices ? slices[k] : 0;
            ub.db[i] = (db && ub.slices[i] > 0) ? db[k] : nullptr;
            const int total = cout[k] * cin[k] * 9 + (ub.slices[i] > 0 ? cout[k] : 0);
            const int epb = 4 * (256 / unpack_groups(total));
            most = std::max(most, (total + epb - 1) / epb);
        }
        const unsigned bx = (unsigned)std::min(most, 2048);
        hipLaunchKernelGGL(unpack_wgrad_batch_kernel, dim3(bx, m), dim3(256), 0, (hipStream_t)stream, ub);
        MMK_LAUNCH_CHECK();
    }
    return MMK_OK;
}

template <int CX, int CG, bool POOLG = false>
int launch_bwd_fused(const BwdFusedArgs &a, int c1, hipStream_t st)
{
    const int spatial = wgrad_slices(CG, CX, c1, a.B, a.H, a.W);
    if (spatial < 1) {
        mmk::set_error("fused backward: occupancy query failed");
        return MMK_ERR_HIP;
    }
    hipLaunchKernelGGL((conv_bwd_fused_kernel<CX, CG, POOLG>), dim3(spatial), dim3(CONV_THREADS), 0, st, a);
    MMK_LAUNCH_CHECK();
    return MMK_OK;
}

extern "C" int mmk_conv_bwd_fused(const void *x, const void *g, const void *wpack_t, float scale, int32_t B, int32_t H, int32_t W,
                                  int32_t C, void *dx, float *partials, int32_t accumulate, void *stream)
{
    MMK_REQUIRE(x && g && wpack_t && dx && partials, "mmk_conv_bwd_fused: NULL pointer");
    MMK_REQUIRE(B >= 1 && H >= 2 && W >= 2 && (C == 8 || C == 16), "mmk_conv_bwd_fused: bad shape (8 or 16 channels)");
    MMK_REQUIRE((size_t)B * H * W * C < ((size_t)1 << 31), "mmk_conv_bwd_fused: tensor too large for 32-bit offsets");
    const BwdFusedArgs a = bwd_fused_args(x, nullptr, g, wpack_t, dx, nullptr, scale, 1, B, H, W, partials, accumulate);
    return C == 8 ? launch_bwd_fused<8, 8>(a, 8, (hipStream_t)stream) : launch_bwd_fused<16, 16>(a, 16, (hipStream_t)stream);
}

extern "C" int mmk_conv_bwd_fused_pooled(const void *x, const void *gy, const void *arg, float pool_scale, const void *wpack_t, float scale,
                                         int32_t B, int32_t H, int32_t W, int32_t C, void *dx, float *partials, int32_t accumulate,
                                         void *stream)
{
    MMK_REQUIRE(x && gy && arg && wpack_t && dx && partials, "mmk_conv_bwd_fused_pooled: NULL pointer");
    MMK_REQUIRE(B >= 1 && H >= 2 && W >= 2 && C == 16, "mmk_conv_bwd_fused_pooled: bad shape (16 channels)");
    MMK_REQUIRE((size_t)B * H * W * C < ((size_t)1 << 31), "mmk_conv_bwd_fused_pooled: tensor too large for 32-bit offsets");
    BwdFusedArgs a = bwd_fused_args(x, nullptr, gy, wpack_t, dx, nullptr, scale, 1, B, H, W, partials, accumulate);
    a.g_arg = (const unsigned *)arg; a.g_scale = pool_scale;
    return launch_bwd_fused<16, 16, true>(a, 16, (hipStream_t)stream);
}

extern "C" int mmk_conv8x16_bwd_fused(const void *x, const void *g, const void *wpack_t, float scale, int32_t B, int32_t H, int32_t W,
                                      void *dx, float *partials, int32_t accumulate, void *stream)
{
    MMK_REQUIRE(x && g && wpack_t && dx && partials, "mmk_conv8x16_bwd_fused: NULL pointer");
    MMK_REQUIRE(B >= 1 && H >= 2 && W >= 2, "mmk_conv8x16_bwd_fused: bad shape");
    MMK_REQUIRE((size_t)B * H * W * 16 < ((size_t)1 << 31), "mmk_conv8x16_bwd_fused: tensor too large for 32-bit offsets");
    BwdFusedArgs a = bwd_fused_args(x, nullptr, g, wpack_t, dx, nullptr, scale, 1, B, H, W, partials, accumulate);
    a.accumulate_dx = 1;
    return launch_bwd_fused<8, 16>(a, 8, (hipStream_t)stream);
}

extern "C" int mmk_conv16x8_bwd_fused(const void *x1, const void *x2, const void *g, const void *wpack_t, float scale, int32_t B,
                                      int32_t H, int32_t W, void *dx1, void *dx2, float *partials, int32_t accumulate, void *stream)
{
    MMK_REQUIRE(x1 && g && wpack_t && dx1 && partials, "mmk_conv16x8_bwd_fused: NULL pointer");
    MMK_REQUIRE((x2 == nullptr) == (dx2 == nullptr), "mmk_conv16x8_bwd_fused: x2 and dx2 go together (both NULL: one 16-channel input / unmasked output)");
    MMK_REQUIRE(B >= 1 && H >= 2 && W >= 2, "mmk_conv16x8_bwd_fused: bad shape");
    MMK_REQUIRE((size_t)B * H * W * 16 < ((size_t)1 << 31), "mmk_conv16x8_bwd_fused: tensor too large for 32-bit offsets");
    const BwdFusedArgs a = bwd_fused_args(x1, x2, g, wpack_t, dx1, dx2, scale, x2 != nullptr, B, H, W, partials, accumulate);
    return launch_bwd_fused<16, 8>(a, x2 ? 8 : 16, (hipStream_t)stream);
}

extern "C" int32_t mmk_conv3x3_wgrad_slices(int32_t cout, int32_t cin, int32_t c1, int32_t B, int32_t H, int32_t W)
{
    if (B < 1 || H < 1 || W < 1 || !chan_ok(cin) || !chan_ok(cout)) return 0;
    const int ns = wgrad_slices(cout, cin, c1, B, H, W);
    return ns < 0 ? 0 : ns;
}

namespace {
int wgrad_partial(const char *who, const void *x1, const void *x2, int C1, int C2, const void *g, const void *arg, float pool_scale,
                  bool pooled, int cout, int B, int H, int W, float *partials, int accumulate, void *stream)
{
    MMK_REQUIRE(x1 && g && partials && (arg || !pooled), "%s: NULL pointer", who);
    MMK_REQUIRE(B >= 1 && H >= (pooled ? 2 : 1) && W >= (pooled ? 2 : 1), "%s: bad shape", who);
    const int cin = C1 + C2;
    MMK_REQUIRE(C1 % 8 == 0 && C2 % 8 == 0 && (C2 == 0 || x2), "%s: bad input split %d+%d", who, C1, C2);
    MMK_REQUIRE(chan_ok(cin) && chan_ok(cout), "%s: unsupported channel counts %d -> %d", who, cin, cout);
    WgradArgs a;
    a.x1 = (const bf16 *)x1; a.x2 = (const bf16 *)x2; a.C1 = C1; a.C2 = C2; a.g = (const bf16 *)g;
    a.B = B; a.H = H; a.W = W; a.CIN = cin; a.COUT = cout;
    a.partials = partials; a.acc_partials = accumulate;
    a.g_arg = (const unsigned *)arg; a.g_scale = pool_scale;
    return dispatch_wgrad(a, (hipStream_t)stream);
}
}

extern "C" int mmk_conv3x3_wgrad_partial(const void *x1, const void *x2, int32_t C1, int32_t C2, const void *g, int32_t cout,
                                         int32_t B, int32_t H, int32_t W, float *partials, int32_t accumulate, void *stream)
{
    return wgrad_partial("mmk_conv3x3_wgrad_partial", x1, x2, C1, C2, g, nullptr, 1.f, false, cout, B, H, W, partials, accumulate, stream);
}

extern "C" int mmk_conv3x3_wgrad_partial_pooled(const void *x1, const void *x2, int32_t C1, int32_t C2, const void *gy, const void *arg,
                                                float pool_scale, int32_t cout, int32_t B, int32_t H, int32_t W, float *partials,
                                                int32_t accumulate, void *stream)
{
    return wgrad_partial("mmk_conv3x3_wgrad_partial_pooled", x1, x2, C1, C2, gy, arg, pool_scale, true, cout, B, H, W, partials, accumulate,
                         stream);
}

extern "C" int mmk_bn_forward_stats(const void *a, int64_t npix, int32_t C, const float *gamma, const float *beta, float eps,
                                    float momentum, float *running_mean, float *running_var, float *part, float *stat, float *affine,
                                    void *stream)
{
    MMK_REQUIRE(a && gamma && beta && part && stat && affine, "mmk_bn_forward_stats: NULL pointer");
    MMK_REQUIRE(npix >= 1 && chan_ok(C) && C <= 2048, "mmk_bn_forward_stats: bad shape (npix %lld, C %d)", (long long)npix, C);
    MMK_REQUIRE((running_mean == nullptr) == (running_var == nullptr), "mmk_bn_forward_stats: running_mean / running_var go together");
    hipStream_t st = (hipStream_t)stream;
    const int per = 256 / (C / 8);
    const int nblk = (int)std::min<int64_t>(BN_BLOCKS, (npix + per - 1) / per);
    hipLaunchKernelGGL(bn_stats_kernel, dim3(nblk), dim3(256), 0, st, (const bf16 *)a, (size_t)npix, C, part);
    MMK_LAUNCH_CHECK();
    hipLaunchKernelGGL(bn_finalize_kernel, dim3((C + 63) / 64), dim3(64), 0, st, part, nblk, C, (double)npix, gamma, beta, eps, momentum,
                       running_mean, running_var, stat, affine);
    MMK_LAUNCH_CHECK();
    return MMK_OK;
}

extern "C" int mmk_bn_apply(const void *a, int64_t npix, int32_t C, const float *affine, float drop_p, uint32_t seed, void *y,
                            void *stream)
{
    MMK_REQUIRE(a && affine && y, "mmk_bn_apply: NULL pointer");
    MMK_REQUIRE(npix >= 1 && chan_ok(C), "mmk_bn_apply: bad shape");
    MMK_REQUIRE(dropout_prob_ok(drop_p), "mmk_bn_apply: dropout probability %g out of range (it is quantised to thr / 65536, thr <= 65535)", (double)drop_p);
    const size_t ngran = (size_t)npix * (C / 8);
    hipLaunchKernelGGL(bn_apply_kernel, dim3((unsigned)std::min<size_t>((ngran + 255) / 256, 8192)), dim3(256), 0, (hipStream_t)stream,
                       (const bf16 *)a, ngran, C, affine, drop_p, seed, (bf16 *)y);
    MMK_LAUNCH_CHECK();
    return MMK_OK;
}

extern "C" int mmk_bn_backward(const void *gd, const void *d, float drop_scale, const void *a, int64_t npix, int32_t C,
                               const float *stat, const float *affine, const float *gamma, float leaky_slope, int32_t accumulate,
                               float *part, float *coef, float *dgamma, float *dbeta, void *gz, void *stream)
{
    MMK_REQUIRE(gd && a && coef && gz, "mmk_bn_backward: NULL pointer");
    MMK_REQUIRE(npix >= 1 && chan_ok(C) && C <= 2048, "mmk_bn_backward: bad shape");
    hipStream_t st = (hipStream_t)stream;
    const size_t ngran = (size_t)npix * (C / 8);
    const unsigned gb = (unsigned)std::min<size_t>((ngran + 255) / 256, 8192);
    if (stat != nullptr) {
        MMK_REQUIRE(gamma && part && dgamma && dbeta, "mmk_bn_backward: NULL pointer (training mode)");
        const int per = 256 / (C / 8);
        const int nblk = (int)std::min<int64_t>(BN_BLOCKS, (npix + per - 1) / per);
        hipLaunchKernelGGL(bn_bwd_reduce_kernel, dim3(nblk), dim3(256), 0, st, (const bf16 *)gd, (const bf16 *)d, drop_scale,
                           (const bf16 *)a, (size_t)npix, C, stat, part);
        MMK_LAUNCH_CHECK();
        hipLaunchKernelGGL(bn_bwd_finalize_kernel, dim3((C + 63) / 64), dim3(64), 0, st, part, nblk, C, (double)npix, gamma, stat,
                           accumulate, coef, dgamma, dbeta);
        MMK_LAUNCH_CHECK();
    } else {
        MMK_REQUIRE(affine != nullptr, "mmk_bn_backward: evaluation mode needs the affine (scale, shift) pairs");
        hipLaunchKernelGGL(bn_eval_coef_kernel, dim3((C + 63) / 64), dim3(64), 0, st, affine, C, coef);
        MMK_LAUNCH_CHECK();
    }
    hipLaunchKernelGGL(bn_bwd_apply_kernel, dim3(gb), dim3(256), 0, st, (const bf16 *)gd, (const bf16 *)d, drop_scale, (const bf16 *)a,
                       ngran, C, stat, coef, leaky_slope, (bf16 *)gz);
    MMK_LAUNCH_CHECK();
    return MMK_OK;
}

static unsigned nblk(size_t n, int t) { return (unsigned)((n + t - 1) / t); }

extern "C" int mmk_channel_minmax(const float *x, int32_t B, int32_t C, int64_t hw, float *part, float *pre, float *minmax,
                                  void *stream)
{
    MMK_REQUIRE(x && part && pre && B >= 1 && C >= 1 && C <= 65535 && hw >= 1, "mmk_channel_minmax: bad argument");
    hipStream_t st = (hipStream_t)stream;
    hipLaunchKernelGGL(channel_minmax_partial_kernel, dim3(MM_BLOCKS, C), dim3(256), 0, st, x, B, C, (size_t)hw, part);
    MMK_LAUNCH_CHECK();
    hipLaunchKernelGGL(channel_minmax_final_kernel, dim3(C), dim3(256), 0, st, part, C, pre, minmax);
    MMK_LAUNCH_CHECK();
    return MMK_OK;
}

extern "C" int mmk_channel_meanstd(const float *x, int32_t B, int32_t C, int64_t hw, double *part, float *pre, void *stream)
{
    MMK_REQUIRE(x && part && pre && B >= 1 && C >= 1 && C <= 65535 && hw >= 1, "mmk_channel_meanstd: bad argument");
    hipStream_t st = (hipStream_t)stream;
    hipLaunchKernelGGL(channel_moment_partial_kernel<false>, dim3(MM_BLOCKS, C), dim3(256), 0, st, x, B, C, (size_t)hw, part);
    MMK_LAUNCH_CHECK();
    hipLaunchKernelGGL(channel_moment_partial_kernel<true>, dim3(MM_BLOCKS, C), dim3(256), 0, st, x, B, C, (size_t)hw, part);
    MMK_LAUNCH_CHECK();
    hipLaunchKernelGGL(channel_meanstd_final_kernel, dim3(C), dim3(256), 0, st, (const double *)part, (size_t)B * (size_t)hw, pre);
    MMK_LAUNCH_CHECK();
    return MMK_OK;
}

extern "C" int mmk_conv_first(const float *x, int32_t cin, const float *W, const float *bias, const float *pre, int32_t B,
                              int32_t H, int32_t Wd, float leaky_slope, void *y, void *stream)
{
    MMK_REQUIRE(x && W && y, "mmk_conv_first: NULL pointer");
    MMK_REQUIRE(leaky_slope >= 0.f && leaky_slope < 1.f, "mmk_conv_first: leaky_slope must be in [0, 1)");
    MMK_REQUIRE(cin >= 1 && cin <= 4 && B >= 1 && H >= 1 && Wd >= 1, "mmk_conv_first: bad shape (cin must be 1..4)");
    const size_t npix = (size_t)B * H * Wd;
    if (Wd % 4 == 0 && npix < (1u << 31)) {
        const unsigned blocks = (unsigned)std::min<size_t>((npix / 4 + 255) / 256, 4096);
        if (leaky_slope > 0.f)
            hipLaunchKernelGGL(conv_first_x4_kernel<true>, dim3(blocks), dim3(256), 0, (hipStream_t)stream, x, cin, W, bias, pre, B, H, Wd,
                               leaky_slope, (bf16 *)y);
        else
            hipLaunchKernelGGL(conv_first_x4_kernel<false>, dim3(blocks), dim3(256), 0, (hipStream_t)stream, x, cin, W, bias, pre, B, H, Wd,
                               leaky_slope, (bf16 *)y);
        MMK_LAUNCH_CHECK();
        return MMK_OK;
    }
    const unsigned blocks = (unsigned)std::min<size_t>((npix + 255) / 256, 8192);
    hipLaunchKernelGGL(conv_first_kernel, dim3(blocks), dim3(256), 0, (hipStream_t)stream, x, cin, W, bias, pre, B, H, Wd, leaky_slope,
                       (bf16 *)y);
    MMK_LAUNCH_CHECK();
    return MMK_OK;
}
// ... 264 lines not shown
```

### mm_masking_amd/csrc/mmk_unet_driver.hip

```cpp
#include <stdlib.h>
#include <string.h>

#include "mmk_common.h"
#include "mmk_unet_shared.h"

namespace {

using mmku::dropout_prob_ok;

constexpr int NCONV = 23;
const int ENC_CH[6] = {8, 16, 32, 64, 128, 256};

struct Tens {
    size_t off = 0;
    int h = 0, w = 0, c = 0;
};

struct Plan {
    int B, H, W, cin;
    int rh[6], rw[6];
    int cout[NCONV], cinn[NCONV];
    Tens a_enc[6], d_enc[6], t[6];
    size_t t_arg[6];
    Tens u[5], a1[5], d1[5], a2[5], d2[5];
// ... 18 lines not shown
        off += bytes;
        return o;
    }
    Tens tens(int B, int h, int w, int c)
    {
        Tens t;
        t.h = h; t.w = w; t.c = c;
        t.off = take((size_t)B * h * w * c * 2);
        return t;
    }
};

bool make_plan(Plan &p, int B, int H, int W, int cin, bool with_scratch)
{
    if (B < 1 || H < 32 || W < 32 || cin < 1 || cin > 4) return false;
    p.B = B; p.H = H; p.W = W; p.cin = cin;
    p.rh[0] = H; p.rw[0] = W;
    for (int i = 1; i < 6; ++i) { p.rh[i] = p.rh[i - 1] / 2; p.rw[i] = p.rw[i - 1] / 2; }
    for (int i = 0; i < 6; ++i) {
        p.cinn[2 * i] = i == 0 ? cin : ENC_CH[i - 1]; p.cout[2 * i] = ENC_CH[i];
        p.cinn[2 * i + 1] = ENC_CH[i]; p.cout[2 * i + 1] = ENC_CH[i];
    }
    for (int j = 0; j < 5; ++j) {
        const int cs = ENC_CH[4 - j];
        p.cinn[12 + 2 * j] = 2 * cs; p.cout[12 + 2 * j] = cs;
        p.cinn[13 + 2 * j] = cs; p.cout[13 + 2 * j] = cs;
    }
    p.cinn[22] = 8; p.cout[22] = 1;
    Bump b;
    for (int k = 1; k <= 21; ++k) {
        const size_t n = mmk_conv3x3_packed_elems(p.cout[k], p.cinn[k], 0);
        if (n == 0) return false;
        p.packs[k] = b.take(n * 2);
    }
    p.a_enc[0] = b.tens(B, H, W, 8);
    p.d_enc[0] = b.tens(B, H, W, 8);
    p.t[0] = p.d_enc[0];
    for (int i = 1; i < 6; ++i) {
        p.a_enc[i] = b.tens(B, p.rh[i - 1], p.rw[i - 1], ENC_CH[i]);
        p.d_enc[i] = b.tens(B, p.rh[i - 1], p.rw[i - 1], ENC_CH[i]);
        p.t[i] = b.tens(B, p.rh[i], p.rw[i], ENC_CH[i]);
        p.t_arg[i] = b.take((size_t)B * p.rh[i] * p.rw[i] * ENC_CH[i] / 2);
    }
    for (int j = 0; j < 5; ++j) {
        const int cs = ENC_CH[4 - j], h = p.rh[4 - j], w = p.rw[4 - j];
        p.u[j] = b.tens(B, h, w, 2 * cs);
        p.a1[j] = b.tens(B, h, w, cs);
        p.d1[j] = b.tens(B, h, w, cs);
        p.a2[j] = b.tens(B, h, w, cs);
        p.d2[j] = b.tens(B, h, w, cs);
    }
    p.mask_raw = b.take((size_t)B * H * W * 4);
    p.amax = b.take((size_t)B * 4);
    p.norm_part = b.take((size_t)B * 64 * 4);
    p.ws_bytes = mmk::align_up(b.off, 256);
    if (!with_scratch) return true;

    Bump s;
    for (int k = 1; k <= 21; ++k) p.packs_t[k] = s.take(mmk_conv3x3_packed_elems(p.cout[k], p.cinn[k], 1) * 2);
    p.gz_final = s.tens(B, H, W, 8);
    for (int j = 0; j < 5; ++j) {
        const int cs = ENC_CH[4 - j], h = p.rh[4 - j], w = p.rw[4 - j];
        p.gz_a2[j] = s.tens(B, h, w, cs);
        p.gsk[j] = s.tens(B, h, w, cs);
        p.gz_d1[j] = s.tens(B, h, w, cs);
        p.gz_a1[j] = s.tens(B, h, w, cs);
        p.g_u[j] = s.tens(B, h, w, 2 * cs);
        p.gz_up[j] = s.tens(B, p.rh[5 - j], p.rw[5 - j], 2 * cs);
    }
    for (int i = 1; i < 6; ++i) {
        p.gz_d[i] = p.g_u[5 - i];
        if (p.gz_d[i].h != p.rh[i - 1] || p.gz_d[i].w != p.rw[i - 1] || p.gz_d[i].c != ENC_CH[i]) return false;
        p.gz_a[i] = s.tens(B, p.rh[i - 1], p.rw[i - 1], ENC_CH[i]);
    }
    p.gz_a[0] = s.tens(B, H, W, 8);
    for (int k = 1; k <= 21; ++k) {
        int h, w, c1;
        if (k < 12) {
            const int i = k / 2;
            h = i == 0 ? H : p.rh[i - 1]; w = i == 0 ? W : p.rw[i - 1];
            c1 = p.cinn[k];
        } else {
            const int j = (k - 12) / 2;
            h = p.rh[4 - j]; w = p.rw[4 - j];
            c1 = p.cinn[k];
        }
        p.slices[k] = mmk_conv3x3_wgrad_slices(p.cout[k], p.cinn[k], c1, B, h, w);
    }
    for (int k = 1; k <= 21; ++k) {
        if (p.slices[k] <= 0) return false;
        p.part[k] = s.take((size_t)(k >= 12 ? 2 : 1) * p.slices[k] * ((size_t)9 * p.cout[k] * p.cinn[k] + p.cout[k]) * 4);
    }
    p.fin_ws = s.take((size_t)B * 130 * 4);
    p.fin_red = s.take((size_t)MMK_FINAL_BWD_WS_FLOATS * 4);
    p.first_ws = s.take(mmk_conv_first_wgrad_ws_bytes(cin));
    p.scratch_bytes = mmk::align_up(s.off, 256);
    return true;
}

inline void *at(void *base, size_t off) { return static_cast<char *>(base) + off; }

#define MMK_TRY(expr)                \
    do {                             \
        const int rc_ = (expr);      \
        if (rc_ != MMK_OK) return rc_; \
    } while (0)

mmk_conv_desc conv_desc(const Plan &p, int h, int w, float slope)
{
    mmk_conv_desc d;
    memset(&d, 0, sizeof(d));
    d.B = p.B; d.H = h; d.W = w; d.leaky_slope = slope;
    d.scale1 = d.scale2 = d.x1_pool_scale = 1.f;
    return d;
}

int pack_all(const Plan &p, const mmk_unet_desc *d, int transposed, void *base, const size_t *offs, void *stream)
{
    const float *Wp[21];
    void *Op[21];
    for (int k = 1; k <= 21; ++k) {
        Wp[k - 1] = d->params[2 * k];
        Op[k - 1] = static_cast<char *>(base) + offs[k];
    }
    return mmk_conv3x3_pack_weights_batch(21, Wp, p.cout + 1, p.cinn + 1, transposed, Op, stream);
}

struct SideStream {
    hipStream_t st = nullptr;
    hipEvent_t fork = nullptr, join = nullptr;
    int dev = -1;
};

bool use_side_stream()
{
    static int v = -1;
    if (v < 0) {
        const char *e = getenv("MMK_UNET_SIDE_STREAM");
        v = (e && e[0] == '0') ? 0 : 1;
    }
    return v == 1;
}

constexpr unsigned POOL_ADJOINT_LEVELS = (1u << 1) | (1u << 2) | (1u << 3) | (1u << 4);
unsigned pool_adjoint_levels()
{
    const unsigned dflt = POOL_ADJOINT_LEVELS;
    const char *e = getenv("MMK_UNET_POOL_ADJOINT");
    if (e == nullptr || e[0] == '\0') return dflt;
    unsigned m = 0;
    for (; *e; ++e)
        if (*e >= '1' && *e <= '5') m |= 1u << (*e - '0');
    return m;
}

int side_stream(SideStream **out)
{
    static thread_local SideStream pool[16];
    int dev = 0;
    MMK_CHECK_HIP(hipGetDevice(&dev));
    SideStream &s = pool[dev & 15];
    if (s.st == nullptr || s.dev != dev) {
        {
            int lo = 0, hi = 0;
            MMK_CHECK_HIP(hipDeviceGetStreamPriorityRange(&lo, &hi));
            MMK_CHECK_HIP(hipStreamCreateWithPriority(&s.st, hipStreamNonBlocking, hi));
        }
        MMK_CHECK_HIP(hipEventCreateWithFlags(&s.fork, hipEventDisableTiming));
        MMK_CHECK_HIP(hipEventCreateWithFlags(&s.join, hipEventDisableTiming));
        s.dev = dev;
    }
    *out = &s;
    return MMK_OK;
}

int check_events(const char *who, void *const *bucket_events)
{
    for (int b = 0; b < MMK_UNET_GRAD_BUCKETS; ++b) MMK_REQUIRE(bucket_events[b] != nullptr, "%s: NULL event %d", who, b);
    return MMK_OK;
}

}

extern "C" size_t mmk_unet_workspace_bytes(int32_t B, int32_t H, int32_t W, int32_t cin)
{
    Plan p;
    if (!make_plan(p, B, H, W, cin, false)) {
        mmk::set_error("mmk_unet_workspace_bytes: unsupported network input (B=%d, %d x %d, %d channels)", B, H, W, cin);
        return 0;
    }
    return p.ws_bytes;
}

extern "C" size_t mmk_unet_scratch_bytes(int32_t B, int32_t H, int32_t W, int32_t cin)
{
    Plan p;
    if (!make_plan(p, B, H, W, cin, true)) {
        mmk::set_error("mmk_unet_scratch_bytes: unsupported network input (B=%d, %d x %d, %d channels)", B, H, W, cin);
        return 0;
    }
    return p.scratch_bytes;
}

extern "C" int mmk_unet_tensor(int32_t B, int32_t H, int32_t W, int32_t cin, int32_t id, size_t *offset, int32_t *h, int32_t *w,
                               int32_t *c)
{
    Plan p;
    MMK_REQUIRE(make_plan(p, B, H, W, cin, false), "mmk_unet_tensor: unsupported network input");
    MMK_REQUIRE(offset && h && w && c, "mmk_unet_tensor: NULL pointer");
    const Tens *t = nullptr;
    if (id >= 0 && id < 6) t = &p.a_enc[id];
    else if (id < 12) t = &p.d_enc[id - 6];
    else if (id < 18) t = &p.t[id - 12];
    else if (id < 18 + 25) {
        const int j = (id - 18) / 5, q = (id - 18) % 5;
        const Tens *arr[5] = {&p.u[j], &p.a1[j], &p.d1[j], &p.a2[j], &p.d2[j]};
        t = arr[q];
    }
    MMK_REQUIRE(t != nullptr, "mmk_unet_tensor: bad tensor id %d", id);
    *offset = t->off; *h = t->h; *w = t->w; *c = t->c;
    return MMK_OK;
}

extern "C" int mmk_unet_forward(const mmk_unet_desc *d, void *stream)
{
    MMK_REQUIRE(d != nullptr, "mmk_unet_forward: NULL descriptor");
    MMK_REQUIRE(d->x && d->params && d->workspace && d->mask, "mmk_unet_forward: NULL pointer");
    Plan p;
    MMK_REQUIRE(make_plan(p, d->B, d->H, d->W, d->cin, false), "mmk_unet_forward: unsupported network input (B=%d, %d x %d, %d channels)",
                d->B, d->H, d->W, d->cin);
    MMK_REQUIRE(d->workspace_bytes >= p.ws_bytes, "mmk_unet_forward: workspace too small (%zu < %zu bytes)", d->workspace_bytes,
                p.ws_bytes);
    MMK_REQUIRE(dropout_prob_ok(d->drop_p), "mmk_unet_forward: dropout probability %g out of range (it is quantised to thr / 65536, thr <= 65535)", (double)d->drop_p);
    for (int i = 0; i < 2 * NCONV; ++i) MMK_REQUIRE(d->params[i] != nullptr, "mmk_unet_forward: NULL parameter %d", i);
    void *ws = d->workspace;
    const float sl = d->leaky_slope;
    const int B = p.B;
    auto Wk = [&](int k) { return d->params[2 * k]; };
    auto Bk = [&](int k) { return d->params[2 * k + 1]; };
    unsigned ctr = d->seed * 64u;
    auto layer = [&](int k, const Tens &x1, const Tens *x2, const Tens &y, bool drop) {
        mmk_conv_desc c = conv_desc(p, y.h, y.w, sl);
        c.x1 = at(ws, x1.off); c.C1 = x1.c; c.wpack = at(ws, p.packs[k]); c.bias = Bk(k);
        if (x2) { c.x2 = at(ws, x2->off); c.C2 = x2->c; }
        c.y1 = at(ws, y.off); c.O1 = y.c; c.relu = 1;
        if (drop) { c.drop_p = d->drop_p; c.seed = ++ctr; }
        return c;
    };
    auto run = [&](const mmk_conv_desc &c) { return mmk_conv3x3(&c, stream); };

    MMK_TRY(pack_all(p, d, 0, ws, p.packs, stream));
    MMK_TRY(mmk_conv_first(d->x, p.cin, Wk(0), Bk(0), d->pre, B, p.H, p.W, sl, at(ws, p.a_enc[0].off), stream));
    MMK_TRY(run(layer(1, p.a_enc[0], nullptr, p.d_enc[0], true)));
    for (int i = 1; i < 6; ++i) {
        const int h = p.rh[i - 1], w = p.rw[i - 1], ch = ENC_CH[i];
        MMK_TRY(run(layer(2 * i, p.t[i - 1], nullptr, p.a_enc[i], false)));
        mmk_conv_desc c2 = layer(2 * i + 1, p.a_enc[i], nullptr, p.d_enc[i], true);
        const bool fuse = sl == 0.f && mmk_conv3x3_pool_fusable(ch, ch, B, h, w) != 0;
        const bool lean = fuse && !d->keep_full_res;
        if (fuse) c2.pool_y = at(ws, p.t[i].off);
        if (lean) { c2.pool_arg = at(ws, p.t_arg[i]); c2.y1 = nullptr; }
        MMK_TRY(run(c2));
        if (sl == 0.f) {
            if (!lean) MMK_TRY(mmk_maxpool2_fwd_arg(at(ws, p.d_enc[i].off), B, h, w, ch, at(ws, p.t[i].off), at(ws, p.t_arg[i]), stream));
        } else {
            MMK_TRY(mmk_maxpool2_fwd(at(ws, p.d_enc[i].off), B, h, w, ch, at(ws, p.t[i].off), stream));
        }
    }
    const Tens *cur = &p.t[5];
    for (int j = 0; j < 5; ++j) {
        const int k0 = 12 + 2 * j, k1 = 13 + 2 * j;
        MMK_TRY(mmk_upsample_fwd(at(ws, cur->off), B, cur->h, cur->w, cur->c, p.u[j].h, p.u[j].w, at(ws, p.u[j].off), stream));
        MMK_TRY(run(layer(k0, p.u[j], nullptr, p.a1[j], false)));
        MMK_TRY(run(layer(k1, p.a1[j], nullptr, p.d1[j], true)));
        MMK_TRY(run(layer(k0, p.t[4 - j], &p.d1[j], p.a2[j], false)));
        MMK_TRY(run(layer(k1, p.a2[j], nullptr, p.d2[j], true)));
        cur = &p.d2[j];
    }
    float *raw = d->norm ? static_cast<float *>(at(ws, p.mask_raw)) : d->mask;
    MMK_TRY(mmk_final_fwd(at(ws, cur->off), Wk(22), Bk(22), (int64_t)B * p.H * p.W, raw, stream));
    if (d->norm)
        MMK_TRY(mmk_mask_normalize(raw, B, (int64_t)p.H * p.W, static_cast<float *>(at(ws, p.norm_part)), d->mask,
                                   static_cast<float *>(at(ws, p.amax)), stream));
    return MMK_OK;
}

namespace {
struct InputGrad {
    float *grad_x;
    int mode;
    const float *minmax;
};
int unet_backward_impl(const mmk_unet_desc *d, const float *gmask, float *const *grads, void *scratch, size_t scratch_bytes,
                       void *const *bucket_events, void *stream, const InputGrad *ig = nullptr);
}

extern "C" int mmk_unet_backward(const mmk_unet_desc *d, const float *gmask, float *const *grads, void *scratch,
                                 size_t scratch_bytes, void *stream)
{
    return unet_backward_impl(d, gmask, grads, scratch, scratch_bytes, nullptr, stream);
}

extern "C" int32_t mmk_unet_grad_bucket(int32_t bucket, int32_t *first_param, int32_t *n_params)
{
    static const int32_t first[MMK_UNET_GRAD_BUCKETS] = {24, 12, 0}, count[MMK_UNET_GRAD_BUCKETS] = {22, 12, 12};
    MMK_REQUIRE(bucket >= 0 && bucket < MMK_UNET_GRAD_BUCKETS && first_param && n_params, "mmk_unet_grad_bucket: bad bucket %d", bucket);
    *first_param = first[bucket];
    *n_params = count[bucket];
    return MMK_OK;
}

extern "C" int mmk_unet_backward_buckets(const mmk_unet_desc *d, const float *gmask, float *const *grads, void *scratch,
                                         size_t scratch_bytes, void *const *bucket_events, void *stream)
{
    MMK_REQUIRE(bucket_events != nullptr, "mmk_unet_backward_buckets: NULL event array");
    MMK_TRY(check_events("mmk_unet_backward_buckets", bucket_events));
    return unet_backward_impl(d, gmask, grads, scratch, scratch_bytes, bucket_events, stream);
}

extern "C" int mmk_unet_backward_input(const mmk_unet_desc *d, const float *gmask, float *const *grads, float *grad_x,
                                       int32_t norm_mode, const float *minmax, void *scratch, size_t scratch_bytes,
                                       void *const *bucket_events, void *stream)
{
    MMK_REQUIRE(d != nullptr, "mmk_unet_backward_input: NULL descriptor");
    MMK_REQUIRE(grad_x != nullptr, "mmk_unet_backward_input: NULL pointer (grad_x)");
    MMK_REQUIRE(d->cin >= 1 && d->cin <= 4, "mmk_unet_backward_input: bad shape (cin must be 1..4)");
    MMK_REQUIRE(norm_mode == MMK_NORM_NONE || norm_mode == MMK_NORM_MINMAX || norm_mode == MMK_NORM_STANDARDIZE,
                "mmk_unet_backward_input: unknown normalisation mode %d", norm_mode);
    MMK_REQUIRE(norm_mode == MMK_NORM_NONE || d->pre != nullptr, "mmk_unet_backward_input: normalisation mode %d needs d->pre (NULL pointer)",
                norm_mode);
    MMK_REQUIRE(norm_mode != MMK_NORM_MINMAX || minmax != nullptr, "mmk_unet_backward_input: MMK_NORM_MINMAX needs minmax (NULL pointer)");
    MMK_REQUIRE(mmk_conv_first_dgrad_ws_bytes(d->cin) <= mmk_conv_first_wgrad_ws_bytes(d->cin),
                "mmk_unet_backward_input: no room for the statistics in scratch");
    if (bucket_events) MMK_TRY(check_events("mmk_unet_backward_input", bucket_events));
    const InputGrad ig = {grad_x, norm_mode, norm_mode == MMK_NORM_MINMAX ? minmax : nullptr};
    return unet_backward_impl(d, gmask, grads, scratch, scratch_bytes, bucket_events, stream, &ig);
}

namespace {
int unet_backward_impl(const mmk_unet_desc *d, const float *gmask, float *const *grads, void *scratch, size_t scratch_bytes,
                       void *const *bucket_events, void *stream, const InputGrad *ig)
{
    MMK_REQUIRE(d != nullptr, "mmk_unet_backward: NULL descriptor");
    MMK_REQUIRE(d->x && d->params && d->workspace && d->mask && gmask && grads && scratch, "mmk_unet_backward: NULL pointer");
    Plan p;
    MMK_REQUIRE(make_plan(p, d->B, d->H, d->W, d->cin, true), "mmk_unet_backward: unsupported network input");
    MMK_REQUIRE(d->workspace_bytes >= p.ws_bytes, "mmk_unet_backward: workspace too small");
    MMK_REQUIRE(scratch_bytes >= p.scratch_bytes, "mmk_unet_backward: scratch too small (%zu < %zu bytes)", scratch_bytes, p.scratch_bytes);
    for (int i = 0; i < 2 * NCONV; ++i) MMK_REQUIRE(d->params[i] && grads[i], "mmk_unet_backward: NULL parameter / gradient %d", i);
    void *ws = d->workspace, *sc = scratch;
    hipStream_t st = (hipStream_t)stream;
    const float sl = d->leaky_slope, s = mmku::dropout_params(d->drop_p).inv_keep;
    const int B = p.B;
    auto Wk = [&](int k) { return d->params[2 * k]; };

    MMK_TRY(pack_all(p, d, 1, sc, p.packs_t, stream));
    SideStream *ss = nullptr;
    if (use_side_stream()) MMK_TRY(side_stream(&ss));
    void *wstream = ss ? (void *)ss->st : stream;
    auto fork = [&]() -> int {
        if (ss) {
            MMK_CHECK_HIP(hipEventRecord(ss->fork, st));
            MMK_CHECK_HIP(hipStreamWaitEvent(ss->st, ss->fork, 0));
        }
        return MMK_OK;
    };
    MMK_TRY(fork());
    int part_used[NCONV] = {};
    auto part_ptr = [&](int k) {
        float *ptr = static_cast<float *>(at(sc, p.part[k])) +
                     (size_t)part_used[k] * p.slices[k] * ((size_t)9 * p.cout[k] * p.cinn[k] + p.cout[k]);
        part_used[k] += 1;
        return ptr;
    };
    auto unpack = [&](int k0, int k1) -> int {
        MMK_TRY(fork());
        const float *src[21];
        int32_t slices[21], co[21], ci[21];
        float *dW[21], *db[21];
        int n = 0;
        for (int k = k0; k <= k1; ++k, ++n) {
            src[n] = static_cast<const float *>(at(sc, p.part[k]));
            if (part_used[k] != (k >= 12 ? 2 : 1)) {
                mmk::set_error("mmk_unet_backward: layer %d wrote %d sets of partial slices", k, part_used[k]);
                return MMK_ERR_ARG;
            }
            slices[n] = p.slices[k] * part_used[k]; co[n] = p.cout[k]; ci[n] = p.cinn[k];
            dW[n] = grads[2 * k]; db[n] = grads[2 * k + 1];
        }
        return mmk_conv3x3_wgrad_unpack_batch(n, src, slices, co, ci, dW, db, wstream);
    };

    auto can_fuse = [&](int k, int ch, int h, int w) {
        return (ch == 8 || ch == 16) && sl == 0.f && p.slices[k] > 0 && mmk_conv3x3_wgrad_slices(ch, ch, ch, B, h, w) == p.slices[k];
    };
    auto bwd_fused = [&](int k, int ch, const void *x, const void *g, void *dx, int h, int w, const void *g_arg = nullptr) -> int {
        if (g_arg) return mmk_conv_bwd_fused_pooled(x, g, g_arg, s, at(sc, p.packs_t[k]), 1.f, B, h, w, ch, dx, part_ptr(k), 0, stream);
        return mmk_conv_bwd_fused(x, g, at(sc, p.packs_t[k]), 1.f, B, h, w, ch, dx, part_ptr(k), 0, stream);
    };
    auto wgrad = [&](int k, const void *x1, int C1, const void *x2, int C2, const void *g, int h, int w, const void *g_arg = nullptr) -> int {
        MMK_TRY(fork());
        if (mmk_conv3x3_wgrad_slices(p.cout[k], p.cinn[k], C1, B, h, w) != p.slices[k]) {
            mmk::set_error("mmk_unet_backward: partial-slice count of layer %d depends on the input split", k);
            return MMK_ERR_ARG;
        }
        if (g_arg) return mmk_conv3x3_wgrad_partial_pooled(x1, x2, C1, C2, g, g_arg, s, p.cout[k], B, h, w, part_ptr(k), 0, wstream);
        return mmk_conv3x3_wgrad_partial(x1, x2, C1, C2, g, p.cout[k], B, h, w, part_ptr(k), 0, wstream);
    };
    auto run = [&](const mmk_conv_desc &c) { return mmk_conv3x3(&c, stream); };
    auto second_conv_bwd = [&](int k, int ch, const void *x, const void *g, void *dx, int h, int w, const void *g_arg) -> int {
        if (can_fuse(k, ch, h, w)) return bwd_fused(k, ch, x, g, dx, h, w, g_arg);
        MMK_TRY(wgrad(k, x, ch, nullptr, 0, g, h, w, g_arg));
        mmk_conv_desc c = conv_desc(p, h, w, sl);
        c.x1 = g; c.C1 = ch; c.wpack = at(sc, p.packs_t[k]); c.y1 = dx; c.O1 = ch; c.relu_src1 = x;
        if (g_arg) { c.x1_pool_arg = g_arg; c.x1_pool_scale = s; }
        return run(c);
    };

    const Tens &d2_4 = p.d2[4];
    if (d->norm)
        MMK_TRY(mmk_final_bwd_normalized(at(ws, d2_4.off), Wk(22), static_cast<const float *>(at(ws, p.mask_raw)), d->mask,
                                         static_cast<const float *>(at(ws, p.amax)), gmask, B, (int64_t)p.H * p.W, s, sl,
                                         static_cast<float *>(at(sc, p.fin_ws)), static_cast<float *>(at(sc, p.fin_ws)) + (size_t)B * 128,
                                         at(sc, p.gz_final.off), grads[44], grads[45], static_cast<float *>(at(sc, p.fin_red)), stream));
    else
        MMK_TRY(mmk_final_bwd(at(ws, d2_4.off), Wk(22), d->mask, gmask, (int64_t)B * p.H * p.W, s, sl, at(sc, p.gz_final.off), grads[44],
                              grads[45], static_cast<float *>(at(sc, p.fin_red)), stream));
    const void *gz = at(sc, p.gz_final.off);
    for (int j = 4; j >= 0; --j) {
        const int cs = ENC_CH[4 - j], h = p.rh[4 - j], w = p.rw[4 - j];
        const int k0 = 12 + 2 * j, k1 = 13 + 2 * j;
        const void *skip = at(ws, p.t[4 - j].off);
        MMK_TRY(second_conv_bwd(k1, cs, at(ws, p.a2[j].off), gz, at(sc, p.gz_a2[j].off), h, w, nullptr));
        if (j == 4 && sl == 0.f && cs == 8 && p.slices[k0] > 0 && mmk_conv3x3_wgrad_slices(8, 16, 8, B, h, w) == p.slices[k0]) {
            MMK_TRY(mmk_conv16x8_bwd_fused(skip, at(ws, p.d1[j].off), at(sc, p.gz_a2[j].off), at(sc, p.packs_t[k0]), s, B, h, w,
                                           at(sc, p.gsk[j].off), at(sc, p.gz_d1[j].off), part_ptr(k0), 0, stream));
        } else {
            MMK_TRY(wgrad(k0, skip, cs, at(ws, p.d1[j].off), cs, at(sc, p.gz_a2[j].off), h, w));
            mmk_conv_desc c2 = conv_desc(p, h, w, sl);
            c2.x1 = at(sc, p.gz_a2[j].off); c2.C1 = cs; c2.wpack = at(sc, p.packs_t[k0]);
            c2.y1 = at(sc, p.gsk[j].off); c2.O1 = cs; c2.scale1 = s;
            c2.relu_src1 = (j == 4) ? skip : nullptr;
            c2.y2 = at(sc, p.gz_d1[j].off); c2.O2 = cs; c2.relu_src2 = at(ws, p.d1[j].off); c2.scale2 = s;
            MMK_TRY(run(c2));
        }
        MMK_TRY(second_conv_bwd(k1, cs, at(ws, p.a1[j].off), at(sc, p.gz_d1[j].off), at(sc, p.gz_a1[j].off), h, w, nullptr));
        if (j == 4 && sl == 0.f && cs == 8 && p.slices[k0] > 0 && mmk_conv3x3_wgrad_slices(8, 16, 16, B, h, w) == p.slices[k0]) {
            MMK_TRY(mmk_conv16x8_bwd_fused(at(ws, p.u[j].off), nullptr, at(sc, p.gz_a1[j].off), at(sc, p.packs_t[k0]), 1.f, B, h, w,
                                           at(sc, p.g_u[j].off), nullptr, part_ptr(k0), 0, stream));
        } else {
            MMK_TRY(wgrad(k0, at(ws, p.u[j].off), 2 * cs, nullptr, 0, at(sc, p.gz_a1[j].off), h, w));
            mmk_conv_desc c4 = conv_desc(p, h, w, sl);
            c4.x1 = at(sc, p.gz_a1[j].off); c4.C1 = cs; c4.wpack = at(sc, p.packs_t[k0]); c4.y1 = at(sc, p.g_u[j].off); c4.O1 = 2 * cs;
            MMK_TRY(run(c4));
        }
        if (j > 0) {
            const Tens &pd2 = p.d2[j - 1];
            MMK_TRY(mmk_upsample_bwd(at(sc, p.g_u[j].off), B, pd2.h, pd2.w, 2 * cs, h, w, at(ws, pd2.off), s, sl, at(sc, p.gz_up[j].off),
                                     stream));
        } else {
            MMK_TRY(mmk_upsample_bwd(at(sc, p.g_u[j].off), B, p.rh[5], p.rw[5], 2 * cs, h, w, nullptr, 1.f, sl, at(sc, p.gz_up[j].off),
                                     stream));
        }
        gz = at(sc, p.gz_up[j].off);
    }
    MMK_TRY(unpack(12, 21));
    if (bucket_events) MMK_CHECK_HIP(hipEventRecord((hipEvent_t)bucket_events[0], (hipStream_t)wstream));
    const unsigned pool_levels = pool_adjoint_levels();
    auto pool_adjoint_fused = [&](int i, int ch) {
        if (!((pool_levels >> i) & 1u)) return false;
        return ch >= 32 || (ch == 16 && can_fuse(2 * i + 1, ch, p.rh[i - 1], p.rw[i - 1]));
    };
    const void *g_t = gz;
    for (int i = 5; i >= 1; --i) {
        const int ch = ENC_CH[i], h = p.rh[i - 1], w = p.rw[i - 1];
        const bool pooled = sl == 0.f && pool_adjoint_fused(i, ch);
        const void *g_d = pooled ? g_t : at(sc, p.gz_d[i].off);
        const void *g_arg = pooled ? at(ws, p.t_arg[i]) : nullptr;
        if (!pooled) {
            if (sl == 0.f)
                MMK_TRY(mmk_maxpool2_bwd_arg(at(ws, p.t_arg[i]), g_t, B, h, w, ch, s, at(sc, p.gz_d[i].off), stream));
            else
                MMK_TRY(mmk_maxpool2_bwd(at(ws, p.d_enc[i].off), g_t, B, h, w, ch, s, sl, at(sc, p.gz_d[i].off), stream));
        }
        MMK_TRY(second_conv_bwd(2 * i + 1, ch, at(ws, p.a_enc[i].off), g_d, at(sc, p.gz_a[i].off), h, w, g_arg));
        void *tgt = at(sc, p.gsk[5 - i].off);
        if (i == 1 && sl == 0.f && ch == 16 && ENC_CH[0] == 8 && p.slices[2] > 0 &&
            mmk_conv3x3_wgrad_slices(16, 8, 8, B, h, w) == p.slices[2]) {
            MMK_TRY(mmk_conv8x16_bwd_fused(at(ws, p.t[0].off), at(sc, p.gz_a[1].off), at(sc, p.packs_t[2]), s, B, h, w, tgt,
                                           part_ptr(2), 0, stream));
        } else {
            MMK_TRY(wgrad(2 * i, at(ws, p.t[i - 1].off), ENC_CH[i - 1], nullptr, 0, at(sc, p.gz_a[i].off), h, w));
            mmk_conv_desc c2 = conv_desc(p, h, w, sl);
            c2.x1 = at(sc, p.gz_a[i].off); c2.C1 = ch; c2.wpack = at(sc, p.packs_t[2 * i]); c2.y1 = tgt; c2.O1 = ENC_CH[i - 1];
            c2.accumulate1 = 1;
            if (i == 1) { c2.relu_src1 = at(ws, p.t[0].off); c2.scale1 = s; }
            MMK_TRY(run(c2));
        }
        g_t = tgt;
        if (i == 3) {
            MMK_TRY(unpack(6, 11));
            if (bucket_events) MMK_CHECK_HIP(hipEventRecord((hipEvent_t)bucket_events[1], (hipStream_t)wstream));
        }
    }
    MMK_TRY(second_conv_bwd(1, 8, at(ws, p.a_enc[0].off), g_t, at(sc, p.gz_a[0].off), p.H, p.W, nullptr));
    MMK_TRY(unpack(1, 5));
    MMK_TRY(mmk_conv_first_wgrad(d->x, p.cin, at(sc, p.gz_a[0].off), d->pre, B, p.H, p.W, grads[0], grads[1],
                                 static_cast<float *>(at(sc, p.first_ws)), mmk_conv_first_wgrad_ws_bytes(p.cin), stream));
    if (ss) {
        MMK_CHECK_HIP(hipEventRecord(ss->join, ss->st));
        MMK_CHECK_HIP(hipStreamWaitEvent(st, ss->join, 0));
    }
    if (bucket_events) MMK_CHECK_HIP(hipEventRecord((hipEvent_t)bucket_events[2], st));
    if (ig) {
        const size_t nws = mmk_conv_first_dgrad_ws_bytes(p.cin);
        void *sws = ig->mode == MMK_NORM_NONE ? nullptr : at(sc, p.first_ws);
        MMK_TRY(mmk_conv_first_dgrad(at(sc, p.gz_a[0].off), p.cin, Wk(0), d->x, d->pre, ig->minmax, B, p.H, p.W, ig->grad_x, sws, nws,
                                     stream));
        MMK_TRY(mmk_input_norm_bwd(ig->grad_x, d->x, p.cin, d->pre, ig->minmax, ig->mode, B, p.H, p.W, sws, nws, stream));
    }
    return MMK_OK;
}
}
```

### mm_masking_amd/unet_hip.py

```python
import ctypes
import os

import torch

from . import _lib

BF16 = torch.bfloat16


def _p(t):
    return None if t is None else ctypes.c_void_p(t.data_ptr())


_sp = _lib.stream_ptr


def _flat_grads(sizes, device):
    offs = [0]
    for n in sizes:
        offs.append(offs[-1] + (n + 3) // 4 * 4)
    flat = torch.zeros(offs[-1], dtype=torch.float32, device=device)
    return flat, [flat[o:o + n] for o, n in zip(offs, sizes)]


def pack_weights(w, transposed=False):
    L = _lib.lib()
    cout, cin = w.shape[0], w.shape[1]
    n = L.mmk_conv3x3_packed_elems(cout, cin, 1 if transposed else 0)
    if n == 0:
        raise _lib.MmkError("unsupported conv channel counts %d -> %d" % (cin, cout))
    out = torch.empty(n, dtype=BF16, device=w.device)
    wf = w.detach().float().contiguous()
    _lib.check(L.mmk_conv3x3_pack_weights(_p(wf), cout, cin, 1 if transposed else 0, _p(out),
                                          _sp(w.device)))
    return out


def pack_weights_batch(ws, transposed=False):
    L = _lib.lib()
    n = len(ws)
    tr = 1 if transposed else 0
    sizes = [L.mmk_conv3x3_packed_elems(w.shape[0], w.shape[1], tr) for w in ws]
    if any(sz == 0 for sz in sizes):
        raise _lib.MmkError("unsupported conv channel counts in pack_weights_batch")
    offs = [0]
    for sz in sizes:
        offs.append(offs[-1] + (sz + 127) // 128 * 128)
    buf = torch.empty(offs[-1], dtype=BF16, device=ws[0].device)
    base = buf.data_ptr()
    wsrc = [w.detach().float().contiguous() for w in ws]
    Wp = (ctypes.c_void_p * n)(*[w.data_ptr() for w in wsrc])
    Op = (ctypes.c_void_p * n)(*[base + 2 * o for o in offs[:-1]])
    co = (ctypes.c_int32 * n)(*[w.shape[0] for w in ws])
    ci = (ctypes.c_int32 * n)(*[w.shape[1] for w in ws])
    _lib.check(L.mmk_conv3x3_pack_weights_batch(n, Wp, co, ci, tr, Op, _sp(ws[0].device)))
    return [buf[offs[i]:offs[i] + sizes[i]] for i in range(n)]


def conv3x3(x1, wpack, cout, bias=None, x2=None, relu=False, drop_p=0.0, seed=0, out=None, out2=None, split=None,
            relu_src=None, scale=1.0, relu_src2=None, scale2=1.0, accumulate=False, accumulate2=False, pool_out=None,
            slope=0.0, pool_arg=None, x1_pool_arg=None, x1_pool_scale=1.0, hw=None):
    B, H, W, C1 = x1.shape
    if x1_pool_arg is not None:
        H, W = hw
        assert x1.shape[1:3] == (H // 2, W // 2) and x1_pool_arg.shape == (B, H // 2, W // 2, C1 // 2)
    C2 = 0 if x2 is None else x2.shape[3]
    O1 = cout if split is None else split
    O2 = cout - O1
    if out is None and pool_arg is None:
        out = torch.empty(B, H, W, O1, dtype=BF16, device=x1.device)
    if O2 > 0 and out2 is None:
        out2 = torch.empty(B, H, W, O2, dtype=BF16, device=x1.device)
    d = _lib.ConvDesc(x1=_p(x1), x2=_p(x2), C1=C1, C2=C2, wpack=_p(wpack), bias=_p(bias), y1=_p(out),
                      relu_src1=_p(relu_src), O1=O1, accumulate1=1 if accumulate else 0, scale1=float(scale),
                      y2=_p(out2), relu_src2=_p(relu_src2), O2=O2, accumulate2=1 if accumulate2 else 0,
                      scale2=float(scale2), B=B, H=H, W=W, relu=1 if relu else 0, leaky_slope=float(slope),
                      drop_p=float(drop_p),
                      seed=int(seed) & 0xFFFFFFFF, pool_y=_p(pool_out), pool_arg=_p(pool_arg), x1_pool_arg=_p(x1_pool_arg),
                      x1_pool_scale=float(x1_pool_scale))
    _lib.check(_lib.lib().mmk_conv3x3(ctypes.byref(d), _sp(x1.device)))
    if pool_arg is not None:
        return None
    return (out, out2) if O2 > 0 else out


def pool_fusable(cin, cout, B, H, W):
    return bool(_lib.lib().mmk_conv3x3_pool_fusable(cin, cout, B, H, W))


def conv3x3_wgrad(x1, g, cout, x2=None, dWt=None, db=None):
    B, H, W, C1 = x1.shape
    C2 = 0 if x2 is None else x2.shape[3]
    cin = C1 + C2
    ns = wgrad_slices(cout, cin, C1, B, H, W)
    if ns <= 0:
        raise _lib.MmkError("conv3x3_wgrad: unsupported shape %d -> %d channels" % (cin, cout))
    part = partial_buffer(ns, cout, cin, x1.device)
    conv3x3_wgrad_partial(x1, g, cout, part, x2=x2)
    tot = part.sum(dim=0)
    w = tot[:9 * cout * cin].view(9, cout, cin)
    if dWt is None:
        dWt = w.clone()
    else:
        dWt += w
    if db is not None:
        db += tot[9 * cout * cin:]
    return dWt


def wgrad_unpack(dWt, accumulate_into=None):
    w = dWt.permute(1, 2, 0).reshape(dWt.shape[1], dWt.shape[2], 3, 3)
    if accumulate_into is not None:
        accumulate_into += w
        return accumulate_into
    return w.contiguous()


def dropout_scale(p):
    f32 = lambda v: ctypes.c_float(v).value
    thr = int(f32(f32(float(p)) * 65536.0 + 0.5))
    return 65536.0 / (65536 - thr) if thr else 1.0


def wgrad_slices(cout, cin, c1, B, H, W):
    return int(_lib.lib().mmk_conv3x3_wgrad_slices(cout, cin, c1, B, H, W))


def partial_buffer(ns, cout, cin, device):
    return torch.empty(ns, 9 * cout * cin + cout, dtype=torch.float32, device=device)


def conv3x3_wgrad_partial(x1, g, cout, partials, x2=None, accumulate=False, g_pool_arg=None, g_pool_scale=1.0):
    B, H, W, C1 = x1.shape
    C2 = 0 if x2 is None else x2.shape[3]
    if g_pool_arg is not None:
        assert g.shape == (B, H // 2, W // 2, cout) and g_pool_arg.shape == (B, H // 2, W // 2, cout // 2)
        _lib.check(_lib.lib().mmk_conv3x3_wgrad_partial_pooled(_p(x1), _p(x2), C1, C2, _p(g), _p(g_pool_arg), float(g_pool_scale),
                                                               cout, B, H, W, _p(partials), 1 if accumulate else 0,
                                                               _sp(x1.device)))
        return partials
    _lib.check(_lib.lib().mmk_conv3x3_wgrad_partial(_p(x1), _p(x2), C1, C2, _p(g), cout, B, H, W, _p(partials),
                                                    1 if accumulate else 0, _sp(x1.device)))
    return partials


def conv_bwd_fused(x, g, wpack_t, scale, dx, partials, accumulate=False, g_pool_arg=None, g_pool_scale=1.0):
    B, H, W, C = x.shape
    if g_pool_arg is not None:
        assert C == 16 and g.shape == (B, H // 2, W // 2, C) and g_pool_arg.shape == (B, H // 2, W // 2, C // 2) and dx.shape == x.shape
        _lib.check(_lib.lib().mmk_conv_bwd_fused_pooled(_p(x), _p(g), _p(g_pool_arg), float(g_pool_scale), _p(wpack_t), float(scale),
                                                        B, H, W, C, _p(dx), _p(partials), 1 if accumulate else 0,
                                                        _sp(x.device)))
        return dx, partials
    assert C in (8, 16) and g.shape == x.shape and dx.shape == x.shape
    _lib.check(_lib.lib().mmk_conv_bwd_fused(_p(x), _p(g), _p(wpack_t), float(scale), B, H, W, C, _p(dx), _p(partials),
                                             1 if accumulate else 0, _sp(x.device)))
    return dx, partials


def conv8x16_bwd_fused(x, g, wpack_t, scale, dx, partials, accumulate=False):
    B, H, W, C = x.shape
    assert C == 8 and g.shape == (B, H, W, 16) and dx.shape == x.shape
    _lib.check(_lib.lib().mmk_conv8x16_bwd_fused(_p(x), _p(g), _p(wpack_t), float(scale), B, H, W, _p(dx), _p(partials),
                                                 1 if accumulate else 0, _sp(x.device)))
    return dx, partials


def conv16x8_bwd_fused(x1, x2, g, wpack_t, scale, dx1, dx2, partials, accumulate=False):
    B, H, W, C = x1.shape
    if x2 is None:
        assert C == 16 and dx2 is None and g.shape == (B, H, W, 8) and dx1.shape == x1.shape
    else:
        assert C == 8 and x2.shape == x1.shape and g.shape == x1.shape and dx1.shape == x1.shape and dx2.shape == x1.shape
    _lib.check(_lib.lib().mmk_conv16x8_bwd_fused(_p(x1), _p(x2), _p(g), _p(wpack_t), float(scale), B, H, W, _p(dx1), _p(dx2),
                                                 _p(partials), 1 if accumulate else 0, _sp(x1.device)))
    return dx1, dx2, partials


def wgrad_unpack_batch(items):
    n = len(items)
    srcs, couts, cins, slices, dbs = [], [], [], [], []
    for it in items:
        if isinstance(it, (tuple, list)):
            t, co, ci = it[0], it[1], it[2]
            srcs.append(t); couts.append(co); cins.append(ci); slices.append(t.shape[0])
            dbs.append(it[3] if len(it) > 3 else None)
        else:
            srcs.append(it); couts.append(it.shape[1]); cins.append(it.shape[2]); slices.append(0); dbs.append(None)
    sizes = [9 * co * ci for co, ci in zip(couts, cins)]
    offs = [0]
    for sz in sizes:
        offs.append(offs[-1] + (sz + 3) // 4 * 4)
    dev = srcs[0].device
    buf = torch.empty(offs[-1], dtype=torch.float32, device=dev)
    base = buf.data_ptr()
    Sp = (ctypes.c_void_p * n)(*[t.data_ptr() for t in srcs])
    Op = (ctypes.c_void_p * n)(*[base + 4 * o for o in offs[:-1]])
    Dp = (ctypes.c_void_p * n)(*[(d.data_ptr() if d is not None else None) for d in dbs])
    sl = (ctypes.c_int32 * n)(*slices)
    co = (ctypes.c_int32 * n)(*couts)
    ci = (ctypes.c_int32 * n)(*cins)
    _lib.check(_lib.lib().mmk_conv3x3_wgrad_unpack_batch(n, Sp, sl, co, ci, Op, Dp, _sp(dev)))
    return [buf[offs[i]:offs[i] + sizes[i]].view(couts[i], cins[i], 3, 3) for i in range(n)]


def conv_first_wgrad(x, gz, pre, dW, db):
    L = _lib.lib()
    B, cin, H, W = x.shape
    nb = int(L.mmk_conv_first_wgrad_ws_bytes(cin))
    ws = torch.empty(nb // 4, dtype=torch.float32, device=x.device)
    _lib.check(L.mmk_conv_first_wgrad(_p(x), cin, _p(gz), _p(pre), B, H, W, _p(dW), _p(db), _p(ws), nb, _sp(x.device)))


def conv_first_dgrad(gz, w, x=None, pre=None, minmax=None, stats=False):
    L = _lib.lib()
    B, H, W, _ = gz.shape
    cin = w.shape[1]
    gx = torch.empty(B, cin, H, W, dtype=torch.float32, device=gz.device)
    ws, nb = None, 0
    if stats:
        nb = int(L.mmk_conv_first_dgrad_ws_bytes(cin))
        ws = torch.empty(nb // 8, dtype=torch.float64, device=gz.device)
    _lib.check(L.mmk_conv_first_dgrad(_p(gz), cin, _p(w), _p(x), _p(pre), _p(minmax), B, H, W, _p(gx), _p(ws), nb, _sp(gz.device)))
    return gx, ws


def input_norm_bwd(gx, x, pre, mode, minmax, ws):
    B, cin, H, W = gx.shape
    _lib.check(_lib.lib().mmk_input_norm_bwd(_p(gx), _p(x), cin, _p(pre), _p(minmax), _lib.NORM_MODES[mode], B, H, W, _p(ws),
                                             0 if ws is None else ws.numel() * 8, _sp(gx.device)))
    return gx


def first_layer_input_grad(x, gz, w, pre, in_norm):
    mode, mm = in_norm if in_norm is not None else (None, None)
    if _lib.NORM_MODES[mode] == 0:
        return conv_first_dgrad(gz, w, pre=pre)[0]
    gx, ws = conv_first_dgrad(gz, w, x=x, pre=pre, minmax=mm if mode == "minmax" else None, stats=True)
    return input_norm_bwd(gx, x, pre, mode, mm, ws)


def conv_first(x, w, b, pre=None, slope=0.0):
    B, cin, H, W = x.shape
    y = torch.empty(B, H, W, 8, dtype=BF16, device=x.device)
    _lib.check(_lib.lib().mmk_conv_first(_p(x), cin, _p(w), _p(b), _p(pre), B, H, W, float(slope), _p(y), _sp(x.device)))
    return y


FORCE_COLLECTIVES = False


def minmax_is_collective(global_reduce, process_group=None):
    from .ddp import dist, job_size
    forced = FORCE_COLLECTIVES and dist.is_available() and dist.is_initialized()
    return bool(global_reduce and (job_size(process_group) > 1 or forced))


def channel_minmax(x, process_group=None, global_reduce=False, return_minmax=False):
    B, C, H, W = x.shape
    part = torch.empty(C * 2048, dtype=torch.float32, device=x.device)
    pre = torch.empty(C, 2, dtype=torch.float32, device=x.device)
    import torch.distributed as dist
    reduce = minmax_is_collective(global_reduce, process_group)
    mm = torch.empty(C, 2, dtype=torch.float32, device=x.device) if (reduce or return_minmax) else None
    _lib.check(_lib.lib().mmk_channel_minmax(_p(x), B, C, H * W, _p(part), _p(pre), _p(mm), _sp(x.device)))
    if reduce:
        t = torch.stack((-mm[:, 0], mm[:, 1]), dim=1)
        dist.all_reduce(t, op=dist.ReduceOp.MAX, group=process_group)
        pre = torch.stack((-t[:, 0], 1.0 / (t[:, 1] + t[:, 0])), dim=1).contiguous()
    return (pre, mm) if return_minmax else pre


def channel_meanstd(x):
    B, C, H, W = x.shape
    part = torch.empty(C * 2048, dtype=torch.float64, device=x.device)
    pre = torch.empty(C, 2, dtype=torch.float32, device=x.device)
    _lib.check(_lib.lib().mmk_channel_meanstd(_p(x), B, C, H * W, _p(part), _p(pre), _sp(x.device)))
    return pre


def maxpool2(x):
    B, H, W, C = x.shape
    y = torch.empty(B, H // 2, W // 2, C, dtype=BF16, device=x.device)
    _lib.check(_lib.lib().mmk_maxpool2_fwd(_p(x), B, H, W, C, _p(y), _sp(x.device)))
    return y


def maxpool2_arg(x):
    B, H, W, C = x.shape
    y = torch.empty(B, H // 2, W // 2, C, dtype=BF16, device=x.device)
    arg = torch.empty(B, H // 2, W // 2, C // 2, dtype=torch.uint8, device=x.device)
    _lib.check(_lib.lib().mmk_maxpool2_fwd_arg(_p(x), B, H, W, C, _p(y), _p(arg), _sp(x.device)))
    return y, arg


def maxpool2_bwd_arg(arg, gy, H, W, scale):
    B, _, _, C = gy.shape
    gz = torch.empty(B, H, W, C, dtype=BF16, device=gy.device)
    _lib.check(_lib.lib().mmk_maxpool2_bwd_arg(_p(arg), _p(gy), B, H, W, C, float(scale), _p(gz), _sp(gy.device)))
    return gz


def maxpool2_bwd(d, gy, scale, slope=0.0):
    B, H, W, C = d.shape
    gz = torch.empty_like(d)
    _lib.check(_lib.lib().mmk_maxpool2_bwd(_p(d), _p(gy), B, H, W, C, float(scale), float(slope), _p(gz), _sp(d.device)))
    return gz


def upsample(x, Ho, Wo):
    B, Hs, Ws, C = x.shape
    y = torch.empty(B, Ho, Wo, C, dtype=BF16, device=x.device)
    _lib.check(_lib.lib().mmk_upsample_fwd(_p(x), B, Hs, Ws, C, Ho, Wo, _p(y), _sp(x.device)))
    return y


def upsample_bwd(gy, Hs, Ws, relu_src=None, scale=1.0, slope=0.0):
    B, Ho, Wo, C = gy.shape
    gx = torch.empty(B, Hs, Ws, C, dtype=BF16, device=gy.device)
    _lib.check(_lib.lib().mmk_upsample_bwd(_p(gy), B, Hs, Ws, C, Ho, Wo, _p(relu_src), float(scale), float(slope),
                                           _p(gx), _sp(gy.device)))
    return gx


def final_fwd(x, w, b):
    B, H, W, _ = x.shape
    mask = torch.empty(B, H, W, dtype=torch.float32, device=x.device)
    _lib.check(_lib.lib().mmk_final_fwd(_p(x), _p(w), _p(b), B * H * W, _p(mask), _sp(x.device)))
# ... 333 lines not shown
```

Before: 3533 pairs/s.

## Extend fused conv backward (dgrad+wgrad) kernel to 32-channel U-Net layers

Generalizes the thin-layer fused backward kernel, which computes input gradient and weight-gradient partials in one pass over shared tiles, to 32-channel inputs and outputs. It adds 32, 16x32 and 32x16 variants, including pooled and concat-split forms. The driver now routes five additional backward sites (enc2, dec2, dec3) through these kernels, gated by an env bitmask that enables all of them by default. The aim is to avoid separate wgrad and dgrad conv launches and the duplicate reads of x and g at these layers. In exchange it raises per-block register and LDS use, which may lower occupancy.

New measurement: 3556 pairs/s (median of 6 runs). Within noise of the previous version (+0.6%).

```diff
diff --git a/include/mmk.h b/include/mmk.h
--- a/include/mmk.h
+++ b/include/mmk.h
@@ -351,6 +351,15 @@
 
 int mmk_conv16x8_bwd_fused(const void *x1, const void *x2, const void *g, const void *wpack_t, float scale, int32_t B, int32_t H,
                            int32_t W, void *dx1, void *dx2, float *partials, int32_t accumulate, void *stream);
+
+int mmk_conv32_bwd_fused(const void *x, const void *g, const void *wpack_t, float scale, int32_t B, int32_t H, int32_t W, void *dx,
+                         float *partials, int32_t accumulate, void *stream);
+int mmk_conv32_bwd_fused_pooled(const void *x, const void *gy, const void *arg, float pool_scale, const void *wpack_t, float scale,
+                                int32_t B, int32_t H, int32_t W, void *dx, float *partials, int32_t accumulate, void *stream);
+int mmk_conv16x32_bwd_fused(const void *x, const void *g, const void *wpack_t, int32_t B, int32_t H, int32_t W, void *dx,
+                            float *partials, int32_t accumulate, void *stream);
+int mmk_conv32x16_bwd_fused(const void *x1, const void *x2, const void *g, const void *wpack_t, float scale, int32_t B, int32_t H,
+                            int32_t W, void *dx1, void *dx2, float *partials, int32_t accumulate, void *stream);
 int mmk_conv3x3_wgrad_unpack_batch(int32_t n, const float *const *src, const int32_t *slices, const int32_t *cout,
                                    const int32_t *cin, float *const *dW, float *const *db, void *stream);
 
diff --git a/mm_masking_amd/_lib.py b/mm_masking_amd/_lib.py
--- a/mm_masking_amd/_lib.py
+++ b/mm_masking_amd/_lib.py
@@ -166,6 +166,10 @@
         "mmk_conv3x3_wgrad_partial_pooled": (ctypes.c_int, [c_vp, c_vp, i32, i32, c_vp, c_vp, f32, i32, i32, i32, i32, c_vp, i32, c_vp]),
         "mmk_conv8x16_bwd_fused": (ctypes.c_int, [c_vp, c_vp, c_vp, ctypes.c_float, i32, i32, i32, c_vp, c_vp, i32, c_vp]),
         "mmk_conv16x8_bwd_fused": (ctypes.c_int, [c_vp, c_vp, c_vp, c_vp, ctypes.c_float, i32, i32, i32, c_vp, c_vp, c_vp, i32, c_vp]),
+        "mmk_conv32_bwd_fused": (ctypes.c_int, [c_vp, c_vp, c_vp, f32, i32, i32, i32, c_vp, c_vp, i32, c_vp]),
+        "mmk_conv32_bwd_fused_pooled": (ctypes.c_int, [c_vp, c_vp, c_vp, f32, c_vp, f32, i32, i32, i32, c_vp, c_vp, i32, c_vp]),
+        "mmk_conv16x32_bwd_fused": (ctypes.c_int, [c_vp, c_vp, c_vp, i32, i32, i32, c_vp, c_vp, i32, c_vp]),
+        "mmk_conv32x16_bwd_fused": (ctypes.c_int, [c_vp, c_vp, c_vp, c_vp, f32, i32, i32, i32, c_vp, c_vp, c_vp, i32, c_vp]),
         "mmk_conv_desc_bytes": (sz, []),
         "mmk_conv3x3_pool_fusable": (ctypes.c_int32, [i32, i32, i32, i32, i32]),
         "mmk_channel_minmax": (ctypes.c_int, [c_vp, i32, i32, ctypes.c_int64, c_vp, c_vp, c_vp, c_vp]),
diff --git a/mm_masking_amd/csrc/mmk_unet.hip b/mm_masking_amd/csrc/mmk_unet.hip
--- a/mm_masking_amd/csrc/mmk_unet.hip
+++ b/mm_masking_amd/csrc/mmk_unet.hip
@@ -1810,15 +1810,19 @@
 template <int CX, int CG, bool POOLG = false>
 __global__ __launch_bounds__(CONV_THREADS) void conv_bwd_fused_kernel(const BwdFusedArgs a)
 {
-    static_assert((CX == 8 || CX == 16) && (CG == 8 || CG == 16), "thin layers");
-    constexpr int NTT = CX == 8 ? 5 : 9;
+    static_assert((CX == 8 || CX == 16 || CX == 32) && (CG == 8 || CG == 16 || CG == 32), "thin layers");
+    constexpr int NTT = CX == 8 ? 5 : 9 * (CX / 16);
     constexpr int NTW = (NTT + 3) / 4;
-    constexpr int NS = CG == 8 ? 3 : 5;
+    constexpr int MTW = CG == 32 ? 2 : 1;
+    constexpr int NS = ksteps(CG);
+    constexpr int MTD = CX == 32 ? 2 : 1;
     constexpr int NT = 4;
     constexpr int GX = CX / 8, GG = CG / 8;
+    constexpr int GXH = GX > 1 ? GX / 2 : 1;
+    constexpr bool ACCX = CX == 16 && CG == 32;
     __shared__ __attribute__((aligned(16))) bf16 x_tile[(HT * WT + 8) * CX];
     __shared__ __attribute__((aligned(16))) bf16 g_tile[(HT * WT + 8) * CG];
-    __shared__ __attribute__((aligned(16))) bf16 w_lds[NS * 64 * 8];
+    __shared__ __attribute__((aligned(16))) bf16 w_lds[NS * MTD * 64 * 8];
 
     const int tid = threadIdx.x, lane = tid & 63;
     const int wv = __builtin_amdgcn_readfirstlane(tid >> 6);
@@ -1828,9 +1832,13 @@
     const int i16 = lane & 15, g4 = lane >> 4, q = i16 >> 2, pp = i16 & 3;
     const bool split = a.x2 != nullptr;
 
-    f32x4 acc[NTW], accb = {0.f, 0.f, 0.f, 0.f};
-#pragma unroll
-    for (int n = 0; n < NTW; ++n) acc[n] = (f32x4){0.f, 0.f, 0.f, 0.f};
+    f32x4 acc[MTW][NTW], accb[MTW];
+#pragma unroll
+    for (int m = 0; m < MTW; ++m) {
+        accb[m] = (f32x4){0.f, 0.f, 0.f, 0.f};
+#pragma unroll
+        for (int n = 0; n < NTW; ++n) acc[m][n] = (f32x4){0.f, 0.f, 0.f, 0.f};
+    }
     bf16x8 ones;
 #pragma unroll
     for (int j = 0; j < 8; ++j) ones[j] = (bf16)1.0f;
@@ -1838,8 +1846,8 @@
 #pragma unroll
     for (int n = 0; n < NTW; ++n) {
         const int nt = wv + 4 * n;
-        int tap = CX == 8 ? 2 * nt + (pp >> 1) : nt;
-        const int col = CX == 8 ? 4 * (pp & 1) : 4 * pp;
+        int tap = CX == 8 ? 2 * nt + (pp >> 1) : nt / (CX >= 16 ? CX / 16 : 1);
+        const int col = CX == 8 ? 4 * (pp & 1) : (nt % (CX >= 16 ? CX / 16 : 1)) * 16 + 4 * pp;
         tap = tap > 8 ? 8 : tap;
         const int ty = tap / 3, tx = tap % 3;
         b_ad[n] = lds_addr(x_tile) + (unsigned)((((ty * WT) + 4 * g4 + q + tx) * CX + col) * 2);
@@ -1849,8 +1857,8 @@
     int d_lane[NS];
 #pragma unroll
     for (int ks = 0; ks < NS; ++ks) {
-        int tap = CG == 8 ? 4 * ks + (lane >> 4) : 2 * ks + (lane >> 5);
-        const int ch = CG == 8 ? 0 : 8 * ((lane >> 4) & 1);
+        int tap, ch;
+        kslot<CG>(ks, lane, tap, ch);
         tap = tap > 8 ? 8 : tap;
         d_lane[ks] = ((2 * wv + tap / 3) * WT + (lane & 15) + tap % 3) * CG + ch;
     }
@@ -1865,9 +1873,17 @@
         o_pix[n] = r * a.W + c;
         s_off[n] = ((r + 1) * WT + c + 1) * CX + (lane >> 4) * 4;
     }
-    bf16 *const o_base = (a.dx2 != nullptr) ? ((lane >> 5) ? a.dx2 : a.dx) + ((lane >> 4) & 1) * 4 : a.dx + (lane >> 4) * 4;
-    const int o_stride = (a.dx2 != nullptr) ? 8 : 16;
-    for (int i = tid; i < NS * 64; i += CONV_THREADS) reinterpret_cast<u32x4 *>(w_lds)[i] = reinterpret_cast<const u32x4 *>(a.wpack_t)[i];
+    bf16 *o_base[MTD];
+    bool o_mask[MTD];
+#pragma unroll
+    for (int m = 0; m < MTD; ++m) {
+        const int c = m * 16 + (lane >> 4) * 4;
+        const bool second = c >= CX / 2;
+        o_base[m] = (a.dx2 != nullptr) ? (second ? a.dx2 : a.dx) + (c & (CX / 2 - 1)) : a.dx + c;
+        o_mask[m] = CX == 32 ? ((a.masked >> ((a.dx2 != nullptr && second) ? 1 : 0)) & 1) != 0 : a.masked != 0;
+    }
+    const int o_stride = (a.dx2 != nullptr) ? CX / 2 : CX;
+    for (int i = tid; i < NS * MTD * 64; i += CONV_THREADS) reinterpret_cast<u32x4 *>(w_lds)[i] = reinterpret_cast<const u32x4 *>(a.wpack_t)[i];
 
     constexpr int NX = HT * WT * GX, NG = HT * WT * GG;
     constexpr int RX = (NX + CONV_THREADS - 1) / CONV_THREADS, RG = (NG + CONV_THREADS - 1) / CONV_THREADS;
@@ -1889,7 +1905,7 @@
             const int dy = pix / WT - 1, dx = pix % WT - 1;
             const bool ok = (unsigned)(ty0 + dy) < (unsigned)a.H && (unsigned)(tx0 + dx) < (unsigned)a.W;
             const long po = pix0 + dy * a.W + dx;
-            const bf16 *src = split ? (half ? a.x2 : a.x) + po * 8 : a.x + po * CX + half * 8;
+            const bf16 *src = split ? (half / GXH ? a.x2 : a.x) + po * (GXH * 8) + (half % GXH) * 8 : a.x + po * CX + half * 8;
             rx[i] = *(ok ? reinterpret_cast<const u32x4 *>(src) : &g_zero16);
         }
         if constexpr (POOLG) {
@@ -1966,6 +1982,15 @@
         const bool ok8 = (ty0 + lrow8) < a.H && (tx0 + lcol8) < a.W;
         u32x4 e8_acc = {0u, 0u, 0u, 0u};
         if constexpr (CX == 8) e8_acc = *((ok8 && a.accumulate_dx) ? reinterpret_cast<const u32x4 *>(a.dx + (long)(pix0 + lpix8) * 8) : &g_zero16);
+        bf16x4 e_acc[ACCX ? NT : 1];
+        if constexpr (ACCX) {
+#pragma unroll
+            for (int n = 0; n < NT; ++n) {
+                const bool okp = (ty0 + 2 * wv + (n >> 1)) < a.H && (tx0 + (n & 1) * 16 + (lane & 15)) < a.W;
+                e_acc[n] = *((okp && a.accumulate_dx) ? reinterpret_cast<const bf16x4 *>(o_base[0] + (long)(pix0 + o_pix[n]) * o_stride)
+                                                      : reinterpret_cast<const bf16x4 *>(&g_zero16));
+            }
+        }
         {
             if (t + t_step < t_end) {
                 ld_tx += adv_tx;
@@ -1979,11 +2004,15 @@
             load_tile(ld_b, ld_ty, ld_tx);
             cb = ld_b; cty = ld_ty; ctx = ld_tx;
         }
-        i32x2 fa[2][2], fb[2][2 * NTW];
+        i32x2 fa[2][2 * MTW], fb[2][2 * NTW];
 #define BF_ISSUE(R, BUF)                                                                     \
     {                                                                                        \
         fa[BUF][0] = tr_read_o<((R) * WT * CG) * 2>(g_ad);                                   \
         fa[BUF][1] = tr_read_o<((R) * WT * CG + 16 * CG) * 2>(g_ad);                         \
+        if constexpr (MTW == 2) {                                                            \
+            fa[BUF][2 * (MTW - 1)] = tr_read_o<((R) * WT * CG + 16) * 2>(g_ad);              \
+            fa[BUF][2 * (MTW - 1) + 1] = tr_read_o<((R) * WT * CG + 16 + 16 * CG) * 2>(g_ad); \
+        }                                                                                    \
         _Pragma("unroll") for (int n = 0; n < NTW; ++n) {                                    \
             fb[BUF][2 * n] = tr_read_o<((R) * WT * CX) * 2>(b_ad[n]);                        \
             fb[BUF][2 * n + 1] = tr_read_o<((R) * WT * CX + 16 * CX) * 2>(b_ad[n]);          \
@@ -1991,10 +2020,12 @@
     }
 #define BF_CONSUME(BUF)                                                                      \
     {                                                                                        \
-        const bf16x8 af = frag_from(fa[BUF][0], fa[BUF][1]);                                 \
-        _Pragma("unroll") for (int n = 0; n < NTW; ++n)                                      \
-            acc[n] = __builtin_amdgcn_mfma_f32_16x16x32_bf16(af, frag_from(fb[BUF][2 * n], fb[BUF][2 * n + 1]), acc[n], 0, 0, 0); \
-        accb = __builtin_amdgcn_mfma_f32_16x16x32_bf16(af, ones, accb, 0, 0, 0);             \
+        _Pragma("unroll") for (int m = 0; m < MTW; ++m) {                                    \
+            const bf16x8 af = frag_from(fa[BUF][2 * m], fa[BUF][2 * m + 1]);                     \
+            _Pragma("unroll") for (int n = 0; n < NTW; ++n)                                  \
+                acc[m][n] = __builtin_amdgcn_mfma_f32_16x16x32_bf16(af, frag_from(fb[BUF][2 * n], fb[BUF][2 * n + 1]), acc[m][n], 0, 0, 0); \
+            accb[m] = __builtin_amdgcn_mfma_f32_16x16x32_bf16(af, ones, accb[m], 0, 0, 0);   \
+        }                                                                                    \
     }
 #define BF_STEP(R)                                                                           \
     {                                                                                        \
@@ -2010,26 +2041,33 @@
 #undef BF_STEP
 #undef BF_CONSUME
 #undef BF_ISSUE
-        f32x4 dacc[NT];
-#pragma unroll
-        for (int n = 0; n < NT; ++n) dacc[n] = (f32x4){0.f, 0.f, 0.f, 0.f};
+        f32x4 dacc[MTD][NT];
+#pragma unroll
+        for (int m = 0; m < MTD; ++m)
+#pragma unroll
+            for (int n = 0; n < NT; ++n) dacc[m][n] = (f32x4){0.f, 0.f, 0.f, 0.f};
 #pragma unroll
         for (int ks = 0; ks < NS; ++ks) {
             const bf16 *bl = g_tile + d_lane[ks];
             bf16x8 bf[NT];
 #pragma unroll
             for (int n = 0; n < NT; ++n) bf[n] = *reinterpret_cast<const bf16x8 *>(bl + ((n >> 1) * WT + (n & 1) * 16) * CG);
-            const bf16x8 af = *reinterpret_cast<const bf16x8 *>(w_lds + ((size_t)(ks * 64 + lane)) * 8);
-#pragma unroll
-            for (int n = 0; n < NT; ++n) dacc[n] = __builtin_amdgcn_mfma_f32_16x16x32_bf16(af, bf[n], dacc[n], 0, 0, 0);
+#pragma unroll
+            for (int m = 0; m < MTD; ++m) {
+                const bf16x8 af = *reinterpret_cast<const bf16x8 *>(w_lds + ((size_t)((ks * MTD + m) * 64 + lane)) * 8);
+#pragma unroll
+                for (int n = 0; n < NT; ++n) dacc[m][n] = __builtin_amdgcn_mfma_f32_16x16x32_bf16(af, bf[n], dacc[m][n], 0, 0, 0);
+            }
         }
         u32x4 e8_src = {0u, 0u, 0u, 0u};
-        bf16x4 e_src[NT];
+        bf16x4 e_src[MTD][NT];
         if constexpr (CX == 8) {
             e8_src = *reinterpret_cast<const u32x4 *>(x_tile + s_off8);
         } else {
 #pragma unroll
-            for (int n = 0; n < NT; ++n) e_src[n] = *reinterpret_cast<const bf16x4 *>(x_tile + s_off[n]);
+            for (int m = 0; m < MTD; ++m)
+#pragma unroll
+                for (int n = 0; n < NT; ++n) e_src[m][n] = *reinterpret_cast<const bf16x4 *>(x_tile + s_off[n] + m * 16);
         }
 #pragma unroll
         for (int i = 0; i < RX; ++i) asm volatile("" : "+v"(rx[i]));
@@ -2043,8 +2081,8 @@
             float v8[8];
 #pragma unroll
             for (int r = 0; r < 4; ++r) {
-                const auto s01 = __builtin_amdgcn_permlane16_swap(__float_as_uint(dacc[0][r]), __float_as_uint(dacc[1][r]), false, false);
-                const auto s23 = __builtin_amdgcn_permlane16_swap(__float_as_uint(dacc[2][r]), __float_as_uint(dacc[3][r]), false, false);
+                const auto s01 = __builtin_amdgcn_permlane16_swap(__float_as_uint(dacc[0][0][r]), __float_as_uint(dacc[0][1][r]), false, false);
+                const auto s23 = __builtin_amdgcn_permlane16_swap(__float_as_uint(dacc[0][2][r]), __float_as_uint(dacc[0][3][r]), false, false);
                 const auto lo = __builtin_amdgcn_permlane32_swap(s01[0], s23[0], false, false);
                 const auto hi = __builtin_amdgcn_permlane32_swap(s01[1], s23[1], false, false);
                 v8[r] = __uint_as_float(lo[0]);
@@ -2065,15 +2103,19 @@
 #pragma unroll
             for (int n = 0; n < NT; ++n) {
                 const bool okp = (ty0 + 2 * wv + (n >> 1)) < a.H && (tx0 + (n & 1) * 16 + (lane & 15)) < a.W;
-                bf16x4 outv;
-#pragma unroll
-                for (int r = 0; r < 4; ++r) {
-                    const float v = fmaxf(dacc[n][r] + 0.f, -INFINITY);
-                    const float masked = ((float)e_src[n][r] > 0.f) ? v * a.scale : 0.f;
-                    outv[r] = (bf16)(a.masked ? masked + 0.f : v);
+#pragma unroll
+                for (int m = 0; m < MTD; ++m) {
+                    bf16x4 outv;
+#pragma unroll
+                    for (int r = 0; r < 4; ++r) {
+                        const float v = fmaxf(dacc[m][n][r] + 0.f, -INFINITY);
+                        const float masked = ((float)e_src[m][n][r] > 0.f) ? v * a.scale : 0.f;
+                        const float tgt = ACCX ? (float)e_acc[ACCX ? n : 0][r] : 0.f;
+                        outv[r] = (bf16)(o_mask[m] ? masked + tgt : (ACCX ? v + tgt : v));
+                    }
+                    bf16x4 *dst = okp ? reinterpret_cast<bf16x4 *>(o_base[m] + (long)(pix0 + o_pix[n]) * o_stride) : reinterpret_cast<bf16x4 *>(g_sink16);
+                    *dst = outv;
                 }
-                bf16x4 *dst = okp ? reinterpret_cast<bf16x4 *>(o_base + (long)(pix0 + o_pix[n]) * o_stride) : reinterpret_cast<bf16x4 *>(g_sink16);
-                *dst = outv;
             }
         }
         if (t + t_step >= t_end) break;
@@ -2084,23 +2126,26 @@
 
     constexpr size_t pstride = (size_t)9 * CG * CX + CG;
 #pragma unroll
-    for (int rr = 0; rr < 4; ++rr) {
-        const int co = g4 * 4 + rr;
-        if (co >= CG) continue;
-#pragma unroll
-        for (int n = 0; n < NTW; ++n) {
-            const int nt = wv + 4 * n;
-            if (nt >= NTT) continue;
-            const int tap = CX == 8 ? 2 * nt + (i16 >> 3) : nt;
-            const int ci = CX == 8 ? (i16 & 7) : i16;
-            if (tap < 9) {
-                float *d = a.partials + (size_t)blockIdx.x * pstride + ((size_t)tap * CG + co) * CX + ci;
-                *d = a.acc_partials ? *d + acc[n][rr] : acc[n][rr];
-            }
-        }
-        if (wv == 0 && i16 == 0) {
-            float *d = a.partials + (size_t)blockIdx.x * pstride + (size_t)9 * CG * CX + co;
-            *d = a.acc_partials ? *d + accb[rr] : accb[rr];
+    for (int m = 0; m < MTW; ++m) {
+#pragma unroll
+        for (int rr = 0; rr < 4; ++rr) {
+            const int co = m * 16 + g4 * 4 + rr;
+            if (co >= CG) continue;
+#pragma unroll
+            for (int n = 0; n < NTW; ++n) {
+                const int nt = wv + 4 * n;
+                if (nt >= NTT) continue;
+                const int tap = CX == 8 ? 2 * nt + (i16 >> 3) : nt / (CX >= 16 ? CX / 16 : 1);
+                const int ci = CX == 8 ? (i16 & 7) : (nt % (CX >= 16 ? CX / 16 : 1)) * 16 + i16;
+                if (tap < 9) {
+                    float *d = a.partials + (size_t)blockIdx.x * pstride + ((size_t)tap * CG + co) * CX + ci;
+                    *d = a.acc_partials ? *d + acc[m][n][rr] : acc[m][n][rr];
+                }
+            }
+            if (wv == 0 && i16 == 0) {
+                float *d = a.partials + (size_t)blockIdx.x * pstride + (size_t)9 * CG * CX + co;
+                *d = a.acc_partials ? *d + accb[m][rr] : accb[m][rr];
+            }
         }
     }
 }
@@ -3938,6 +3983,28 @@
     return launch_bwd_fused<16, 16, true>(a, 16, (hipStream_t)stream);
 }
 
+extern "C" int mmk_conv32_bwd_fused(const void *x, const void *g, const void *wpack_t, float scale, int32_t B, int32_t H, int32_t W,
+                                    void *dx, float *partials, int32_t accumulate, void *stream)
+{
+    MMK_REQUIRE(x && g && wpack_t && dx && partials, "mmk_conv32_bwd_fused: NULL pointer");
+    MMK_REQUIRE(B >= 1 && H >= 2 && W >= 2, "mmk_conv32_bwd_fused: bad shape");
+    MMK_REQUIRE((size_t)B * H * W * 32 < ((size_t)1 << 31), "mmk_conv32_bwd_fused: tensor too large for 32-bit offsets");
+    const BwdFusedArgs a = bwd_fused_args(x, nullptr, g, wpack_t, dx, nullptr, scale, 1, B, H, W, partials, accumulate);
+    return launch_bwd_fused<32, 32>(a, 32, (hipStream_t)stream);
+}
+
+extern "C" int mmk_conv32_bwd_fused_pooled(const void *x, const void *gy, const void *arg, float pool_scale, const void *wpack_t,
+                                           float scale, int32_t B, int32_t H, int32_t W, void *dx, float *partials, int32_t accumulate,
+                                           void *stream)
+{
+    MMK_REQUIRE(x && gy && arg && wpack_t && dx && partials, "mmk_conv32_bwd_fused_pooled: NULL pointer");
+    MMK_REQUIRE(B >= 1 && H >= 2 && W >= 2, "mmk_conv32_bwd_fused_pooled: bad shape");
+    MMK_REQUIRE((size_t)B * H * W * 32 < ((size_t)1 << 31), "mmk_conv32_bwd_fused_pooled: tensor too large for 32-bit offsets");
+    BwdFusedArgs a = bwd_fused_args(x, nullptr, gy, wpack_t, dx, nullptr, scale, 1, B, H, W, partials, accumulate);
+    a.g_arg = (const unsigned *)arg; a.g_scale = pool_scale;
+    return launch_bwd_fused<32, 32, true>(a, 32, (hipStream_t)stream);
+}
+
 extern "C" int mmk_conv8x16_bwd_fused(const void *x, const void *g, const void *wpack_t, float scale, int32_t B, int32_t H, int32_t W,
                                       void *dx, float *partials, int32_t accumulate, void *stream)
 {
@@ -3958,6 +4025,28 @@
     MMK_REQUIRE((size_t)B * H * W * 16 < ((size_t)1 << 31), "mmk_conv16x8_bwd_fused: tensor too large for 32-bit offsets");
     const BwdFusedArgs a = bwd_fused_args(x1, x2, g, wpack_t, dx1, dx2, scale, x2 != nullptr, B, H, W, partials, accumulate);
     return launch_bwd_fused<16, 8>(a, x2 ? 8 : 16, (hipStream_t)stream);
+}
+
+extern "C" int mmk_conv16x32_bwd_fused(const void *x, const void *g, const void *wpack_t, int32_t B, int32_t H, int32_t W, void *dx,
+                                       float *partials, int32_t accumulate, void *stream)
+{
+    MMK_REQUIRE(x && g && wpack_t && dx && partials, "mmk_conv16x32_bwd_fused: NULL pointer");
+    MMK_REQUIRE(B >= 1 && H >= 2 && W >= 2, "mmk_conv16x32_bwd_fused: bad shape");
+    MMK_REQUIRE((size_t)B * H * W * 32 < ((size_t)1 << 31), "mmk_conv16x32_bwd_fused: tensor too large for 32-bit offsets");
+    BwdFusedArgs a = bwd_fused_args(x, nullptr, g, wpack_t, dx, nullptr, 1.f, 0, B, H, W, partials, accumulate);
+    a.accumulate_dx = 1;
+    return launch_bwd_fused<16, 32>(a, 16, (hipStream_t)stream);
+}
+
+extern "C" int mmk_conv32x16_bwd_fused(const void *x1, const void *x2, const void *g, const void *wpack_t, float scale, int32_t B,
+                                       int32_t H, int32_t W, void *dx1, void *dx2, float *partials, int32_t accumulate, void *stream)
+{
+    MMK_REQUIRE(x1 && g && wpack_t && dx1 && partials, "mmk_conv32x16_bwd_fused: NULL pointer");
+    MMK_REQUIRE((x2 == nullptr) == (dx2 == nullptr), "mmk_conv32x16_bwd_fused: x2 and dx2 go together (both NULL: one 32-channel input / unmasked output)");
+    MMK_REQUIRE(B >= 1 && H >= 2 && W >= 2, "mmk_conv32x16_bwd_fused: bad shape");
+    MMK_REQUIRE((size_t)B * H * W * 32 < ((size_t)1 << 31), "mmk_conv32x16_bwd_fused: tensor too large for 32-bit offsets");
+    const BwdFusedArgs a = bwd_fused_args(x1, x2, g, wpack_t, dx1, dx2, scale, x2 ? 2 : 0, B, H, W, partials, accumulate);
+    return launch_bwd_fused<32, 16>(a, x2 ? 16 : 32, (hipStream_t)stream);
 }
 
 extern "C" int32_t mmk_conv3x3_wgrad_slices(int32_t cout, int32_t cin, int32_t c1, int32_t B, int32_t H, int32_t W)
diff --git a/mm_masking_amd/csrc/mmk_unet_driver.hip b/mm_masking_amd/csrc/mmk_unet_driver.hip
--- a/mm_masking_amd/csrc/mmk_unet_driver.hip
+++ b/mm_masking_amd/csrc/mmk_unet_driver.hip
@@ -194,6 +194,21 @@
     for (; *e; ++e)
         if (*e >= '1' && *e <= '5') m |= 1u << (*e - '0');
     return m;
+}
+
+enum : unsigned {
+    FUSED32_DEC2_2 = 1u << 0,
+    FUSED32_ENC2_2 = 1u << 1,
+    FUSED32_ENC2_0 = 1u << 2,
+    FUSED32_DEC3_0_UP = 1u << 3,
+    FUSED32_DEC3_0_CAT = 1u << 4,
+};
+constexpr unsigned BWD_FUSED32_SITES = FUSED32_DEC2_2 | FUSED32_ENC2_2 | FUSED32_ENC2_0 | FUSED32_DEC3_0_UP | FUSED32_DEC3_0_CAT;
+unsigned bwd_fused32_sites()
+{
+    const char *e = getenv("MMK_UNET_BWD_FUSED32");
+    if (e == nullptr || e[0] == '\0') return BWD_FUSED32_SITES;
+    return (unsigned)strtoul(e, nullptr, 0) & 0x1fu;
 }
 
 int side_stream(SideStream **out)
@@ -433,10 +448,19 @@
         return mmk_conv3x3_wgrad_unpack_batch(n, src, slices, co, ci, dW, db, wstream);
     };
 
+    const unsigned fused32 = bwd_fused32_sites();
     auto can_fuse = [&](int k, int ch, int h, int w) {
-        return (ch == 8 || ch == 16) && sl == 0.f && p.slices[k] > 0 && mmk_conv3x3_wgrad_slices(ch, ch, ch, B, h, w) == p.slices[k];
+        const bool has = ch == 8 || ch == 16 || (ch == 32 && (fused32 & (k == 5 ? FUSED32_ENC2_2 : FUSED32_DEC2_2)));
+        return has && sl == 0.f && p.slices[k] > 0 && mmk_conv3x3_wgrad_slices(ch, ch, ch, B, h, w) == p.slices[k];
+    };
+    auto can_fuse_first = [&](int k, int cout, int cin, int c1, int h, int w) {
+        return sl == 0.f && p.slices[k] > 0 && mmk_conv3x3_wgrad_slices(cout, cin, c1, B, h, w) == p.slices[k];
     };
     auto bwd_fused = [&](int k, int ch, const void *x, const void *g, void *dx, int h, int w, const void *g_arg = nullptr) -> int {
+        if (ch == 32) {
+            if (g_arg) return mmk_conv32_bwd_fused_pooled(x, g, g_arg, s, at(sc, p.packs_t[k]), 1.f, B, h, w, dx, part_ptr(k), 0, stream);
+            return mmk_conv32_bwd_fused(x, g, at(sc, p.packs_t[k]), 1.f, B, h, w, dx, part_ptr(k), 0, stream);
+        }
         if (g_arg) return mmk_conv_bwd_fused_pooled(x, g, g_arg, s, at(sc, p.packs_t[k]), 1.f, B, h, w, ch, dx, part_ptr(k), 0, stream);
         return mmk_conv_bwd_fused(x, g, at(sc, p.packs_t[k]), 1.f, B, h, w, ch, dx, part_ptr(k), 0, stream);
     };
@@ -477,6 +501,9 @@
         if (j == 4 && sl == 0.f && cs == 8 && p.slices[k0] > 0 && mmk_conv3x3_wgrad_slices(8, 16, 8, B, h, w) == p.slices[k0]) {
             MMK_TRY(mmk_conv16x8_bwd_fused(skip, at(ws, p.d1[j].off), at(sc, p.gz_a2[j].off), at(sc, p.packs_t[k0]), s, B, h, w,
                                            at(sc, p.gsk[j].off), at(sc, p.gz_d1[j].off), part_ptr(k0), 0, stream));
+        } else if (cs == 16 && (fused32 & FUSED32_DEC3_0_CAT) && can_fuse_first(k0, 16, 32, 16, h, w)) {
+            MMK_TRY(mmk_conv32x16_bwd_fused(skip, at(ws, p.d1[j].off), at(sc, p.gz_a2[j].off), at(sc, p.packs_t[k0]), s, B, h, w,
+                                            at(sc, p.gsk[j].off), at(sc, p.gz_d1[j].off), part_ptr(k0), 0, stream));
         } else {
             MMK_TRY(wgrad(k0, skip, cs, at(ws, p.d1[j].off), cs, at(sc, p.gz_a2[j].off), h, w));
             mmk_conv_desc c2 = conv_desc(p, h, w, sl);
@@ -490,6 +517,9 @@
         if (j == 4 && sl == 0.f && cs == 8 && p.slices[k0] > 0 && mmk_conv3x3_wgrad_slices(8, 16, 16, B, h, w) == p.slices[k0]) {
             MMK_TRY(mmk_conv16x8_bwd_fused(at(ws, p.u[j].off), nullptr, at(sc, p.gz_a1[j].off), at(sc, p.packs_t[k0]), 1.f, B, h, w,
                                            at(sc, p.g_u[j].off), nullptr, part_ptr(k0), 0, stream));
+        } else if (cs == 16 && (fused32 & FUSED32_DEC3_0_UP) && can_fuse_first(k0, 16, 32, 32, h, w)) {
+            MMK_TRY(mmk_conv32x16_bwd_fused(at(ws, p.u[j].off), nullptr, at(sc, p.gz_a1[j].off), at(sc, p.packs_t[k0]), 1.f, B, h, w,
+                                            at(sc, p.g_u[j].off), nullptr, part_ptr(k0), 0, stream));
         } else {
             MMK_TRY(wgrad(k0, at(ws, p.u[j].off), 2 * cs, nullptr, 0, at(sc, p.gz_a1[j].off), h, w));
             mmk_conv_desc c4 = conv_desc(p, h, w, sl);
@@ -531,6 +561,9 @@
             mmk_conv3x3_wgrad_slices(16, 8, 8, B, h, w) == p.slices[2]) {
             MMK_TRY(mmk_conv8x16_bwd_fused(at(ws, p.t[0].off), at(sc, p.gz_a[1].off), at(sc, p.packs_t[2]), s, B, h, w, tgt,
                                            part_ptr(2), 0, stream));
+        } else if (i == 2 && ch == 32 && ENC_CH[1] == 16 && (fused32 & FUSED32_ENC2_0) && can_fuse_first(4, 32, 16, 16, h, w)) {
+            MMK_TRY(mmk_conv16x32_bwd_fused(at(ws, p.t[1].off), at(sc, p.gz_a[2].off), at(sc, p.packs_t[4]), B, h, w, tgt, part_ptr(4), 0,
+                                            stream));
         } else {
             MMK_TRY(wgrad(2 * i, at(ws, p.t[i - 1].off), ENC_CH[i - 1], nullptr, 0, at(sc, p.gz_a[i].off), h, w));
             mmk_conv_desc c2 = conv_desc(p, h, w, sl);
diff --git a/mm_masking_amd/unet_hip.py b/mm_masking_amd/unet_hip.py
--- a/mm_masking_amd/unet_hip.py
+++ b/mm_masking_amd/unet_hip.py
@@ -174,6 +174,39 @@
         assert C == 8 and x2.shape == x1.shape and g.shape == x1.shape and dx1.shape == x1.shape and dx2.shape == x1.shape
     _lib.check(_lib.lib().mmk_conv16x8_bwd_fused(_p(x1), _p(x2), _p(g), _p(wpack_t), float(scale), B, H, W, _p(dx1), _p(dx2),
                                                  _p(partials), 1 if accumulate else 0, _sp(x1.device)))
+    return dx1, dx2, partials
+
+
+def conv32_bwd_fused(x, g, wpack_t, scale, dx, partials, accumulate=False, g_pool_arg=None, g_pool_scale=1.0):
+    B, H, W, C = x.shape
+    assert C == 32 and dx.shape == x.shape
+    if g_pool_arg is not None:
+        assert g.shape == (B, H // 2, W // 2, C) and g_pool_arg.shape == (B, H // 2, W // 2, C // 2)
+        _lib.check(_lib.lib().mmk_conv32_bwd_fused_pooled(_p(x), _p(g), _p(g_pool_arg), float(g_pool_scale), _p(wpack_t), float(scale),
+                                                          B, H, W, _p(dx), _p(partials), 1 if accumulate else 0, _sp(x.device)))
+        return dx, partials
+    assert g.shape == x.shape
+    _lib.check(_lib.lib().mmk_conv32_bwd_fused(_p(x), _p(g), _p(wpack_t), float(scale), B, H, W, _p(dx), _p(partials),
+                                               1 if accumulate else 0, _sp(x.device)))
+    return dx, partials
+
+
+def conv16x32_bwd_fused(x, g, wpack_t, dx, partials, accumulate=False):
+    B, H, W, C = x.shape
+    assert C == 16 and g.shape == (B, H, W, 32) and dx.shape == x.shape
+    _lib.check(_lib.lib().mmk_conv16x32_bwd_fused(_p(x), _p(g), _p(wpack_t), B, H, W, _p(dx), _p(partials),
+                                                  1 if accumulate else 0, _sp(x.device)))
+    return dx, partials
+
+
+def conv32x16_bwd_fused(x1, x2, g, wpack_t, scale, dx1, dx2, partials, accumulate=False):
+    B, H, W, C = x1.shape
+    if x2 is None:
+        assert C == 32 and dx2 is None and g.shape == (B, H, W, 16) and dx1.shape == x1.shape
+    else:
+        assert C == 16 and x2.shape == x1.shape and g.shape == x1.shape and dx1.shape == x1.shape and dx2.shape == x1.shape
+    _lib.check(_lib.lib().mmk_conv32x16_bwd_fused(_p(x1), _p(x2), _p(g), _p(wpack_t), float(scale), B, H, W, _p(dx1), _p(dx2),
+                                                  _p(partials), 1 if accumulate else 0, _sp(x1.device)))
     return dx1, dx2, partials
 
 
```
